# kpreid/all-is-cubes

Measured on AMD Instinct MI355X. Metric: Mrays/s, higher is better.
Workload: dtype f64

## Files before the change

### all_is_cubes_amd/abi.py

```python
from __future__ import annotations

import ctypes as C
import math
from pathlib import Path
from typing import Optional

import numpy as np

_PKG = Path(__file__).resolve().parent
LIB_PATH = _PKG / "libaic_hip.so"

AIC_OK = 0
ERR_NAMES = {1: "AIC_ERR_INVALID", 2: "AIC_ERR_NO_DEVICE", 3: "AIC_ERR_OOM", 4: "AIC_ERR_DEVICE", 5: "AIC_ERR_UNSUPPORTED"}
LAYER_WORLD, LAYER_UI = 0, 1
MAX_IN_FLIGHT = 32
FLAW_UNSUPPORTED, FLAW_NO_BLOOM = 1, 2
FRAME_COUNTERS, FRAME_AUX, FRAME_PIXEL_CENTERS, FRAME_OUT_LINEAR, FRAME_OUT_COLORBUF, FRAME_NO_FEEDBACK = 1, 2, 4, 8, 16, 32
FRAME_BLOOM = 64
RAYS_NO_SKY, RAYS_DEVICE = 128, 256
MAX_RAYS = 2048 * 65535
TUNE_QUEUES_SHIFT, TUNE_SUPER_SHIFT, TUNE_VARIANT_SHIFT = 0, 4, 9
VARIANT_AUTO, VARIANT_PLAIN, VARIANT_EXCHANGING, VARIANT_RECORDING = 0, 1, 2, 3
LIGHT_HOOK_SESSION, LIGHT_HOOK_POOL_SHIFT = 1, 8


def bloom_geometry(width: int, height: int):
    rx, ry = (width + 1) // 2, (height + 1) // 2
    levels = min(6, min(rx, ry).bit_length())
    d = 1 << levels
    return levels, ((rx + d - 1) // d * d, (ry + d - 1) // d * d)


def tuning(queues=None, super_shift=None, variant=None) -> int:
    t = 0
    if queues is not None:
        t |= (int(queues) & 15) << TUNE_QUEUES_SHIFT
    if super_shift is not None:
        t |= ((int(super_shift) + 1) & 31) << TUNE_SUPER_SHIFT
    if variant is not None:
        t |= (int(variant) & 3) << TUNE_VARIANT_SHIFT
    return t

ABI_SYMBOLS = [
    "aic_abi_version", "aic_create", "aic_destroy", "aic_last_error", "aic_device_name", "aic_upload_space",
    "aic_clear_space", "aic_update_cubes", "aic_update_light_volume", "aic_replace_block", "aic_replace_blocks", "aic_compact", "aic_set_options",
    "aic_render", "aic_render_submit", "aic_render_wait", "aic_render_submit_batch", "aic_render_wait_batch", "aic_trace_patches", "aic_trace_rays", "aic_partition_rows", "aic_assemble_strips", "aic_assemble_strips_async", "aic_assemble_strips_on", "aic_read_aux", "aic_synchronize", "aic_stream", "aic_wait_event", "aic_stream_wait_frame",
    "aic_probe_raycast", "aic_probe_light_lut", "aic_probe_powf", "aic_probe_expf", "aic_probe_bloom",
    "aic_ortho_image_size", "aic_render_orthographic",
    "aic_evaluate_light", "aic_evaluate_light_submit", "aic_evaluate_light_wait", "aic_evaluate_light_poll", "aic_light_cubes_changed", "aic_read_light_volume", "aic_read_light_cubes", "aic_light_chart", "aic_probe_derived", "aic_probe_log2f",
    "aic_create_multi", "aic_destroy_multi", "aic_multi_device_count", "aic_multi_context", "aic_multi_last_error", "aic_multi_upload_space",
    "aic_multi_clear_space", "aic_multi_update_cubes", "aic_multi_update_light_volume", "aic_multi_evaluate_light", "aic_multi_light_cubes_changed", "aic_multi_replace_blocks", "aic_multi_set_options",
    "aic_multi_render", "aic_multi_render_submit", "aic_multi_render_wait",
]


class AicError(RuntimeError):

    def __init__(self, code: int, message: str):
        super().__init__(f"{ERR_NAMES.get(code, code)}: {message}")
        self.code = code


class BlockDesc(C.Structure):
    _fields_ = [("resolution", C.c_int32), ("vlo", C.c_int32 * 3), ("vsize", C.c_int32 * 3), ("vox_off", C.c_uint32),
                ("pal_off", C.c_uint32), ("pal_len", C.c_uint32), ("flags", C.c_uint32), ("reserved", C.c_int32)]


class LightParams(C.Structure):
    _fields_ = [("maximum_distance", C.c_int32), ("fast", C.c_int32), ("epsilon", C.c_int32), ("batch", C.c_int32),
                ("queue_order", C.c_int32), ("n_queue", C.c_int32), ("lanes_per_cube", C.c_int32), ("hooks", C.c_int32), ("queue_cubes", C.c_void_p), ("queue_priorities", C.c_void_p),
                ("max_updates", C.c_uint64)]


class LightInfo(C.Structure):
    _fields_ = [("updates", C.c_uint64), ("batches", C.c_uint64), ("cost", C.c_uint64), ("device_ms", C.c_double),
                ("total_ms", C.c_double), ("queue_left", C.c_uint32), ("pad", C.c_uint32), ("bundles_visited", C.c_uint64)]


def light_chart():
    lib = load()
    lib.aic_light_chart.restype = C.c_uint32
    lib.aic_light_chart.argtypes = [C.c_void_p, C.c_void_p, C.POINTER(C.c_uint32)]
    depth = C.c_uint32(0)
    n = lib.aic_light_chart(None, None, C.byref(depth))
    w = np.zeros((n, 6), np.float32)
    ch = np.zeros((n, 6), np.uint32)
    lib.aic_light_chart(w.ctypes.data, ch.ctypes.data, C.byref(depth))
    return w, ch, int(depth.value)


class SpaceDesc(C.Structure):
    _fields_ = [("lo", C.c_int32 * 3), ("size", C.c_int32 * 3), ("block_index", C.c_void_p), ("light", C.c_void_p),
                ("n_blocks", C.c_uint32), ("blocks", C.c_void_p), ("voxels", C.c_void_p), ("n_voxels", C.c_uint64),
                ("palette", C.c_void_p), ("n_palette", C.c_uint64), ("sky_kind", C.c_int32), ("sky", (C.c_float * 3) * 8),
                ("block_sky", (C.c_uint8 * 4) * 7)]


class Options(C.Structure):
    _fields_ = [("fog", C.c_int32), ("transparency", C.c_int32), ("threshold", C.c_float), ("lighting", C.c_int32),
                ("bounce_samples", C.c_int32), ("antialiasing", C.c_int32), ("debug_pixel_cost", C.c_int32),
                ("tone_mapping", C.c_int32), ("maximum_intensity", C.c_float), ("bloom_intensity", C.c_float),
                ("view_distance", C.c_double)]


class Camera(C.Structure):
    _fields_ = [("inverse_projection_view", C.c_double * 16), ("exposure", C.c_float), ("reserved", C.c_int32)]


class Partition(C.Structure):
    _fields_ = [("strip_rows", C.c_uint32), ("n_parts", C.c_uint32), ("part", C.c_uint32), ("reserved", C.c_uint32)]


class FrameDesc(C.Structure):
    _fields_ = [("width", C.c_uint32), ("height", C.c_uint32), ("world", Camera), ("ui", Camera), ("backdrop", C.c_float * 4),
                ("partition", Partition), ("flags", C.c_uint32), ("tuning", C.c_uint32)]


class FrameInfo(C.Structure):
    _fields_ = [("cubes_traced", C.c_uint64), ("n_outer", C.c_uint64), ("n_inner", C.c_uint64), ("n_hits", C.c_uint64),
                ("n_light", C.c_uint64), ("kernel_ms", C.c_float), ("total_ms", C.c_float), ("rows_rendered", C.c_uint32),
                ("flaws", C.c_uint32), ("variant", C.c_uint32), ("tile_queues", C.c_uint32)]


PIXEL_AUX_DTYPE = np.dtype(
    [("hit", "<i4"), ("cube", "<i4", (3,)), ("voxel", "<i4", (3,)), ("resolution", "<i4"), ("face", "<i4"),
     ("block_index", "<i4"), ("cubes_traced", "<u4"), ("layer", "<u4"), ("t_distance", "<f8")],
    align=True,
)
RC_STEP_DTYPE = np.dtype([("cube", "<i4", (3,)), ("face", "<i4"), ("t_distance", "<f8"), ("intersection_point", "<f8", (3,))], align=True)

_lib: Optional[C.CDLL] = None


def load() -> C.CDLL:
    global _lib
    if _lib is None:
        if not LIB_PATH.exists():
            raise ImportError(f"{LIB_PATH} is missing: build it with __graft_entry__.build() (hipcc, gfx950)")
        try:
            import torch
        except ImportError:
            pass
        lib = C.CDLL(str(LIB_PATH))
        lib.aic_create.restype = C.c_void_p
        lib.aic_create.argtypes = [C.c_int, C.POINTER(C.c_int)]
        lib.aic_destroy.argtypes = [C.c_void_p]
        lib.aic_destroy.restype = None
        lib.aic_last_error.restype = C.c_char_p
        lib.aic_last_error.argtypes = [C.c_void_p]
        lib.aic_stream.restype = C.c_void_p
        lib.aic_stream.argtypes = [C.c_void_p]
        lib.aic_partition_rows.restype = C.c_uint32
        lib.aic_partition_rows.argtypes = [C.c_uint32, C.POINTER(Partition)]
        lib.aic_upload_space.argtypes = [C.c_void_p, C.c_int, C.POINTER(SpaceDesc)]
        lib.aic_clear_space.argtypes = [C.c_void_p, C.c_int]
        lib.aic_compact.argtypes = [C.c_void_p, C.c_int]
        lib.aic_update_cubes.argtypes = [C.c_void_p, C.c_int, C.c_uint32, C.c_void_p, C.c_void_p, C.c_void_p]
        lib.aic_update_light_volume.argtypes = [C.c_void_p, C.c_int, C.c_void_p]
        lib.aic_replace_block.argtypes = [C.c_void_p, C.c_int, C.c_uint32, C.POINTER(BlockDesc), C.c_void_p, C.c_void_p]
        lib.aic_replace_blocks.argtypes = [C.c_void_p, C.c_int, C.c_uint32, C.c_void_p, C.c_void_p, C.c_void_p, C.c_void_p]
        lib.aic_set_options.argtypes = [C.c_void_p, C.c_int, C.POINTER(Options)]
        lib.aic_render.argtypes = [C.c_void_p, C.POINTER(FrameDesc), C.c_void_p, C.c_int, C.POINTER(FrameInfo)]
        lib.aic_render_submit.argtypes = [C.c_void_p, C.POINTER(FrameDesc), C.c_void_p, C.c_uint32]
        lib.aic_render_wait.argtypes = [C.c_void_p, C.c_uint32, C.POINTER(FrameInfo)]
        lib.aic_render_submit_batch.argtypes = [C.c_void_p, C.c_uint32, C.POINTER(FrameDesc), C.POINTER(C.c_void_p), C.c_uint32]
        lib.aic_render_wait_batch.argtypes = [C.c_void_p, C.c_uint32, C.c_uint32, C.POINTER(FrameInfo)]
        lib.aic_trace_patches.argtypes = [C.c_void_p, C.POINTER(FrameDesc), C.c_uint32, C.c_void_p, C.c_void_p, C.c_void_p, C.POINTER(FrameInfo)]
        lib.aic_trace_rays.argtypes = [C.c_void_p, C.c_int, C.c_uint32, C.c_void_p, C.c_uint32, C.c_float, C.c_void_p, C.c_void_p, C.POINTER(FrameInfo)]
        lib.aic_assemble_strips.argtypes = [C.c_void_p, C.c_void_p, C.c_void_p, C.c_uint32, C.c_uint32, C.c_uint32, C.c_uint32]
        lib.aic_assemble_strips_async.argtypes = [C.c_void_p, C.c_void_p, C.c_void_p, C.c_uint32, C.c_uint32, C.c_uint32, C.c_uint32]
        lib.aic_read_aux.argtypes = [C.c_void_p, C.c_void_p, C.c_uint64]
        lib.aic_synchronize.argtypes = [C.c_void_p]
        lib.aic_wait_event.argtypes = [C.c_void_p, C.c_void_p]
        lib.aic_stream_wait_frame.argtypes = [C.c_void_p, C.c_uint32, C.c_void_p]
        lib.aic_device_name.argtypes = [C.c_void_p, C.c_char_p, C.c_uint32]
        lib.aic_probe_raycast.argtypes = [C.c_void_p, C.c_void_p, C.c_void_p, C.c_int, C.c_void_p, C.c_void_p, C.c_int,
                                          C.c_uint32, C.c_void_p, C.POINTER(C.c_uint32), C.POINTER(C.c_int)]
        lib.aic_probe_light_lut.argtypes = [C.c_void_p, C.c_void_p]
        lib.aic_probe_powf.argtypes = [C.c_void_p, C.c_void_p, C.c_void_p, C.c_uint32, C.c_void_p]
        lib.aic_probe_expf.argtypes = [C.c_void_p, C.c_void_p, C.c_uint32, C.c_void_p]
        lib.aic_probe_bloom.argtypes = [C.c_void_p, C.c_uint32, C.c_uint32, C.c_void_p, C.c_float, C.POINTER(Options), C.c_void_p, C.c_void_p,
                                        C.POINTER(C.c_uint32 * 2)]
        lib.aic_evaluate_light.argtypes = [C.c_void_p, C.c_int, C.POINTER(LightParams), C.POINTER(LightInfo)]
        lib.aic_evaluate_light_submit.argtypes = [C.c_void_p, C.c_int, C.POINTER(LightParams)]
        lib.aic_evaluate_light_wait.argtypes = [C.c_void_p, C.c_int, C.POINTER(LightInfo)]
        lib.aic_evaluate_light_poll.argtypes = [C.c_void_p, C.c_int, C.POINTER(C.c_int)]
        lib.aic_read_light_volume.argtypes = [C.c_void_p, C.c_int, C.c_void_p]
        lib.aic_read_light_cubes.argtypes = [C.c_void_p, C.c_int, C.c_uint32, C.c_void_p, C.c_void_p]
        lib.aic_light_cubes_changed.argtypes = [C.c_void_p, C.c_int, C.c_uint32, C.c_void_p, C.c_int]
        lib.aic_probe_derived.argtypes = [C.c_void_p, C.c_int, C.c_void_p, C.c_void_p]
        lib.aic_probe_log2f.argtypes = [C.c_void_p, C.c_void_p, C.c_uint32, C.c_void_p]
        assert C.sizeof(BlockDesc) == 48
        _lib = lib
    return _lib


def packed_light_scalar_in(value: float) -> int:
    v = np.float32(value)
    if not v > 0:
        return 0
    x = float(np.float32(np.float32(np.log2(v)) * np.float32(10.0)) + np.float32(144.0))
    x = float(np.float32(x))
    r = math.floor(abs(x) + 0.5) * (1 if x >= 0 else -1)
    return int(min(max(r, 0), 255))


def block_sky_texels(sky_kind: int, sky: np.ndarray) -> np.ndarray:
    sky = np.asarray(sky, np.float32).reshape(8, 3)
    out = np.zeros((7, 4), np.uint8)
    out[:, 3] = 255

    def some(rgb):
        return [packed_light_scalar_in(float(c)) for c in rgb]

    if sky_kind == 0:
        out[:, 0:3] = some(sky[0])
        return out
    bases = {
        0: ((0, 1, 0), (0, 0, 1), (1, 0, 0)),
        1: ((0, 0, 1), (1, 0, 0), (0, 1, 0)),
        2: ((1, 0, 0), (0, 1, 0), (0, 0, 1)),
        3: ((0, -1, 0), (0, 0, 1), (-1, 0, 0)),
        4: ((0, 0, 1), (-1, 0, 0), (0, -1, 0)),
        5: ((1, 0, 0), (0, -1, 0), (0, 0, -1)),
    }
    pts = [(-1, -1, -1), (-1, 1, -1), (1, -1, -1), (1, 1, -1)]
    for f in range(6):
        bx, by, bz = (np.array(v) for v in bases[f])
        acc = np.zeros(3, np.float32)
        for p in pts:
            d = p[0] * bx + p[1] * by + p[2] * bz
            idx = ((1 if d[0] >= 0 else 0) << 2) + ((1 if d[1] >= 0 else 0) << 1) + (1 if d[2] >= 0 else 0)
            acc = (acc + sky[idx]).astype(np.float32)
        out[f, 0:3] = some(acc * np.float32(0.25))
    acc = np.zeros(3, np.float32)
    for k in range(8):
        acc = (acc + sky[k]).astype(np.float32)
    out[6, 0:3] = some(acc * np.float32(1.0 / 8.0))
    return out


def make_options(fog=1, transparency=1, threshold=0.5, lighting=3, bounce_samples=0, antialiasing=0, debug_pixel_cost=False,
                 tone_mapping=0, maximum_intensity=float("inf"), bloom_intensity=0.125, view_distance=200.0) -> Options:
    o = Options()
    o.fog, o.transparency, o.threshold, o.lighting = fog, transparency, threshold, lighting
    o.bounce_samples, o.antialiasing, o.debug_pixel_cost = bounce_samples, antialiasing, int(debug_pixel_cost)
    o.tone_mapping, o.maximum_intensity, o.bloom_intensity = tone_mapping, maximum_intensity, bloom_intensity
    o.view_distance = min(max(view_distance, 1.0), 10000.0)
    return o


def unaltered_colors(**kw) -> Options:
    base = dict(fog=0, lighting=0, transparency=1, bloom_intensity=0.0)
    base.update(kw)
    return make_options(**base)


def _ptr(a: Optional[np.ndarray]):
    return None if a is None or a.size == 0 else a.ctypes.data


# ... 259 lines not shown
            raise ValueError("colorbuf must be [h][w][4]")
        h, w = cb.shape[:2]
        out = np.zeros((h, w, 4), np.uint8)
        size = (C.c_uint32 * 2)()
        t0 = bloom_geometry(w, h)[1]
        mip0 = np.zeros((t0[1], t0[0], 4), np.float16) if want_mip0 else None
        self._check(self._lib.aic_probe_bloom(self._h, w, h, _ptr(cb), float(exposure), C.byref(options), _ptr(out),
                                              _ptr(mip0) if mip0 is not None else None, C.byref(size)))
        assert (size[0], size[1]) == t0, ((size[0], size[1]), t0)
        return (out, mip0) if want_mip0 else out

    def evaluate_light(self, layer: int, maximum_distance: int, fast: bool = True, epsilon: int = 1, batch: int = 32,
                       queue_order: int = 16, queue=None, max_updates: int = 0, lanes_per_cube: int = 0, session: bool = False,
                       dep_pool_chunks: int = 0) -> LightInfo:
        hooks = (LIGHT_HOOK_SESSION if session else 0) | ((int(dep_pool_chunks) & 0xffff) << LIGHT_HOOK_POOL_SHIFT)
        p = LightParams(maximum_distance, int(fast), epsilon, batch, queue_order, -1, lanes_per_cube, hooks, None, None, max_updates)
        keep = []
        if queue is not None:
            qc = np.ascontiguousarray([q[0] for q in queue], np.int32).reshape(-1, 3)
            qp = np.ascontiguousarray([q[1] for q in queue], np.int32)
            keep = [qc, qp]
            p.n_queue = len(qp)
            p.queue_cubes = qc.ctypes.data
            p.queue_priorities = qp.ctypes.data
        info = LightInfo()
        self._check(self._lib.aic_evaluate_light(self._h, layer, C.byref(p), C.byref(info)))
        del keep
        return info

    def evaluate_light_submit(self, layer: int, maximum_distance: int, fast: bool = True, epsilon: int = 1, batch: int = 32, queue_order: int = 16,
                              queue=None, max_updates: int = 0, lanes_per_cube: int = 0) -> None:
        p = LightParams(maximum_distance, int(fast), epsilon, batch, queue_order, -1, lanes_per_cube, 0, None, None, max_updates)
        keep = []
        if queue is not None:
            qc = np.ascontiguousarray([q[0] for q in queue], np.int32).reshape(-1, 3)
            qp = np.ascontiguousarray([q[1] for q in queue], np.int32)
            keep = [qc, qp]
            p.n_queue = len(qp)
            p.queue_cubes = qc.ctypes.data
            p.queue_priorities = qp.ctypes.data
        self._check(self._lib.aic_evaluate_light_submit(self._h, layer, C.byref(p)))
        del keep

    def evaluate_light_done(self, layer: int) -> bool:
        d = C.c_int(1)
        self._check(self._lib.aic_evaluate_light_poll(self._h, layer, C.byref(d)))
        return bool(d.value)

    def evaluate_light_wait(self, layer: int) -> LightInfo:
        info = LightInfo()
        self._check(self._lib.aic_evaluate_light_wait(self._h, layer, C.byref(info)))
        return info

    def light_cubes_changed(self, layer: int, xyz, queue_order: int = 16) -> None:
        xyz = np.ascontiguousarray(xyz, np.int32).reshape(-1, 3)
        self._check(self._lib.aic_light_cubes_changed(self._h, layer, len(xyz), _ptr(xyz), queue_order))

    def read_light_volume(self, layer: int, shape) -> np.ndarray:
        out = np.zeros(tuple(shape) + (4,), np.uint8)
        self._check(self._lib.aic_read_light_volume(self._h, layer, out.ctypes.data))
        return out

    def read_light_cubes(self, layer: int, xyz) -> np.ndarray:
        xyz = np.ascontiguousarray(xyz, np.int32).reshape(-1, 3)
        out = np.zeros((len(xyz), 4), np.uint8)
        self._check(self._lib.aic_read_light_cubes(self._h, layer, len(xyz), _ptr(xyz), out.ctypes.data))
        return out

    def probe_derived(self, layer: int, n_blocks: int):
        out = np.zeros((n_blocks, 32), np.float32)
        opq = np.zeros((n_blocks, 6), np.uint8)
        self._check(self._lib.aic_probe_derived(self._h, layer, out.ctypes.data, opq.ctypes.data))
        return out, opq

    def probe_log2f(self, x) -> np.ndarray:
        x = np.ascontiguousarray(x, np.float32)
        out = np.zeros(x.shape, np.float32)
        self._check(self._lib.aic_probe_log2f(self._h, _ptr(x), x.size, _ptr(out)))
        return out

    def probe_light_lut(self) -> np.ndarray:
        out = np.zeros(256, np.float32)
        self._check(self._lib.aic_probe_light_lut(self._h, out.ctypes.data))
        return out


class MultiContext:

    def __init__(self, device_ids):
        self._lib = load()
        lib = self._lib
        lib.aic_create_multi.restype = C.c_void_p
        lib.aic_create_multi.argtypes = [C.c_int, C.c_void_p, C.POINTER(C.c_int)]
        lib.aic_destroy_multi.argtypes = [C.c_void_p]
        lib.aic_multi_last_error.restype = C.c_char_p
        lib.aic_multi_last_error.argtypes = [C.c_void_p]
        lib.aic_multi_device_count.argtypes = [C.c_void_p]
        lib.aic_multi_upload_space.argtypes = [C.c_void_p, C.c_int, C.c_void_p]
        lib.aic_multi_clear_space.argtypes = [C.c_void_p, C.c_int]
        lib.aic_multi_set_options.argtypes = [C.c_void_p, C.c_int, C.c_void_p]
        lib.aic_multi_update_light_volume.argtypes = [C.c_void_p, C.c_int, C.c_void_p]
        lib.aic_multi_evaluate_light.argtypes = [C.c_void_p, C.c_int, C.POINTER(LightParams), C.POINTER(LightInfo)]
        lib.aic_multi_light_cubes_changed.argtypes = [C.c_void_p, C.c_int, C.c_uint32, C.c_void_p, C.c_int]
        lib.aic_multi_update_cubes.argtypes = [C.c_void_p, C.c_int, C.c_uint32, C.c_void_p, C.c_void_p, C.c_void_p]
        lib.aic_multi_render.argtypes = [C.c_void_p, C.c_void_p, C.c_void_p, C.c_int, C.c_void_p]
        lib.aic_multi_render_submit.argtypes = [C.c_void_p, C.c_void_p, C.c_void_p, C.c_int, C.c_uint32]
        lib.aic_multi_render_wait.argtypes = [C.c_void_p, C.c_uint32, C.c_void_p]
        ids = np.ascontiguousarray(device_ids, np.int32)
        st = C.c_int(0)
        self._h = lib.aic_create_multi(len(ids), _ptr(ids), C.byref(st))
        if not self._h:
            raise AicError(st.value, "aic_create_multi failed (no usable MI355X?)")

    def close(self) -> None:
        if self._h:
            self._lib.aic_destroy_multi(self._h)
            self._h = None

    def __enter__(self):
        return self

    def __exit__(self, *exc):
        self.close()

    def _check(self, rc: int) -> None:
        if rc != AIC_OK:
            raise AicError(rc, self._lib.aic_multi_last_error(self._h).decode())

    @property
    def device_count(self) -> int:
        return int(self._lib.aic_multi_device_count(self._h))

    def upload_space(self, layer: int, flat_space) -> None:
        d, _keep = Context._space_desc(flat_space)
        self._check(self._lib.aic_multi_upload_space(self._h, layer, C.byref(d)))

    def clear_space(self, layer: int) -> None:
        self._check(self._lib.aic_multi_clear_space(self._h, layer))

    def set_options(self, layer: int, options: Options) -> None:
        self._check(self._lib.aic_multi_set_options(self._h, layer, C.byref(options)))

    def update_light_volume(self, layer: int, light) -> None:
        lt = np.ascontiguousarray(light, np.uint8)
        self._check(self._lib.aic_multi_update_light_volume(self._h, layer, _ptr(lt)))

    def evaluate_light(self, layer: int, maximum_distance: int, fast: bool = True, epsilon: int = 1, batch: int = 32, queue_order: int = 16) -> LightInfo:
        p = LightParams(maximum_distance, int(fast), epsilon, batch, queue_order, -1, 0, 0, None, None, 0)
        info = LightInfo()
        self._check(self._lib.aic_multi_evaluate_light(self._h, layer, C.byref(p), C.byref(info)))
        return info

    def light_cubes_changed(self, layer: int, xyz, queue_order: int = 16) -> None:
        xyz = np.ascontiguousarray(xyz, np.int32).reshape(-1, 3)
        self._check(self._lib.aic_multi_light_cubes_changed(self._h, layer, len(xyz), _ptr(xyz), queue_order))

    def update_cubes(self, layer: int, xyz, block_index=None, light=None) -> None:
        xyz = np.ascontiguousarray(xyz, np.int32).reshape(-1, 3)
        bi = None if block_index is None else np.ascontiguousarray(block_index, np.uint16)
        lt = None if light is None else np.ascontiguousarray(light, np.uint8).reshape(-1, 4)
        self._check(self._lib.aic_multi_update_cubes(self._h, layer, len(xyz), _ptr(xyz), _ptr(bi), _ptr(lt)))

    def render(self, frame: FrameDesc):
        out = np.zeros((frame.height, frame.width, 4), np.uint8)
        info = FrameInfo()
        self._check(self._lib.aic_multi_render(self._h, C.byref(frame), _ptr(out), 0, C.byref(info)))
# ... 12 lines not shown
```

### all_is_cubes_amd/csrc/aic_abi.cpp

```cpp

#include <hip/hip_runtime.h>

#include <chrono>
#include <cmath>
#include <condition_variable>
#include <mutex>
#include <thread>
#include <cstdio>
#include <cstdlib>
#include <cstring>
#include <initializer_list>
#include <string>
#include <utility>
#include <vector>

#include "../../include/aic_hip.h"
#include "aic_bloom.h"
#include "aic_ctx.h"
#include "aic_device.h"

namespace aic {
void launch_trace_image(const DevFrame &F, bool diag, hipStream_t stream);
size_t trace_ray_cold_bytes(uint32_t n_cus, uint32_t *groups);
void launch_scatter_cubes(uint16_t *grid, uint32_t *light, const int32_t *xyz, const uint16_t *bi, const uint32_t *lt,
                          uint32_t n, const int lo[3], const int size[3], const uint32_t *cls, hipStream_t stream);
void launch_probe_powf(const float *x, const float *y, float *out, uint32_t n, hipStream_t stream);
void launch_probe_expf(const float *x, float *out, uint32_t n, hipStream_t stream);
void launch_order_tiles(const uint32_t *cost, uint32_t *order, uint32_t n_tiles, uint32_t macros_x, uint32_t sb_shift, uint32_t n_queues, uint32_t *queue_start,
                        hipStream_t stream, bool clear_cost = false, uint32_t *clear_words = nullptr, uint32_t n_clear_words = 0);
void launch_order_tiles_jobs(const OrderJobs &jobs, uint32_t n_jobs, uint32_t n_tiles, uint32_t macros_x, uint32_t sb_shift, uint32_t n_queues, hipStream_t stream,
                             bool clear_cost, uint32_t n_clear_words);
void launch_tag_cubes(uint16_t *grid, size_t n, const uint32_t *cls, int from_tagged, int to_tagged, hipStream_t stream);
void launch_assemble_strips(const uint32_t *gathered, uint32_t *out, uint32_t w, uint32_t h, uint32_t strip_rows,
                            uint32_t n_parts, uint32_t max_rows, hipStream_t stream);
void launch_probe_raycast(const double *od, int use_bounds, const int *lohi, int include_exit, uint32_t max_steps,
                          double *out_rec, uint32_t *n_out, int *ended, hipStream_t stream);
}

using namespace aic;

static_assert(sizeof(aic_pixel_aux) == sizeof(DevAux), "aux record layout");

static_assert(sizeof(aic_block_desc) == 48, "aic_block_desc is 48 bytes");

namespace {

constexpr uint64_t kMaxPoolElems = 0x7ffffff0ull;
constexpr uint64_t kMaxLightTexels = 0x3ffffff0ull;

aic_options default_options() {
    aic_options o;
    std::memset(&o, 0, sizeof(o));
    o.fog = 1;
    o.transparency = 1;
    o.threshold = 0.5f;
    o.lighting = 3;
    o.maximum_intensity = INFINITY;
    o.bloom_intensity = 0.125f;
    o.view_distance = 200.0;
    return o;
}

enum DumpTag : uint32_t { DUMP_UPLOAD = 1, DUMP_CLEAR = 2, DUMP_CUBES = 3, DUMP_LIGHT = 4, DUMP_BLOCK = 5, DUMP_OPTIONS = 6, DUMP_FRAME = 7 };
struct DumpPart { const void *p; size_t n; };
void dump_record(aic_ctx *c, uint32_t tag, uint32_t layer, std::initializer_list<DumpPart> parts) {
    if (!c || !c->dump) return;
    uint64_t total = 0;
    for (const DumpPart &d : parts) total += d.p ? d.n : 0;
    std::fwrite(&tag, 4, 1, c->dump);
    std::fwrite(&layer, 4, 1, c->dump);
    std::fwrite(&total, 8, 1, c->dump);
    for (const DumpPart &d : parts)
        if (d.p && d.n) std::fwrite(d.p, 1, d.n, c->dump);
    std::fflush(c->dump);
}

}

namespace aic {

thread_local std::string *tl_err_sink = nullptr;
int fail(aic_ctx *c, int code, const char *what, hipError_t e) {
    if (c) {
        std::string &dst = tl_err_sink ? *tl_err_sink : c->err;
        dst = what;
        if (e != hipSuccess) {
            dst += ": ";
            dst += hipGetErrorString(e);
        }
    }
    return code;
}

int hip_fail(aic_ctx *c, const char *what, hipError_t e) {
    return fail(c, e == hipErrorOutOfMemory ? AIC_ERR_OOM : AIC_ERR_DEVICE, what, e);
}

int take_light_spare(aic_ctx *c, Layer &l, int layer, size_t n, int *index) {
    auto in_use = [&](const DevBuf<uint32_t> &b) {
        for (uint32_t i = 0; i < AIC_MAX_IN_FLIGHT; i++)
            if (c->slots[i].busy && b.p && c->slots[i].light_used[layer] == (const void *)b.p) return true;
        return false;
    };
    int pick = -1;
    for (int k = 0; k < Layer::kLightSpares && pick < 0; k++)
        if (l.light_spare[k].p && l.light_spare[k].cap >= n && !in_use(l.light_spare[k])) pick = k;
    for (int k = 0; k < Layer::kLightSpares && pick < 0; k++)
        if (!l.light_spare[k].p || (l.light_spare[k].cap < n && !in_use(l.light_spare[k]))) pick = k;
    if (pick < 0) {
        pick = 0;
        for (uint32_t i = 0; i < AIC_MAX_IN_FLIGHT; i++)
            if (c->slots[i].busy && c->slots[i].light_used[layer] == (const void *)l.light_spare[0].p) {
                const hipError_t e = hipStreamSynchronize(c->slots[i].stream);
                if (e != hipSuccess) return fail(c, AIC_ERR_DEVICE, "waiting for a frame that reads a spare light volume", e);
            }
    }
    const hipError_t e = l.light_spare[pick].ensure(n);
    if (e != hipSuccess) return fail(c, e == hipErrorOutOfMemory ? AIC_ERR_OOM : AIC_ERR_DEVICE, "alloc light (spare volume)", e);
    *index = pick;
    return AIC_OK;
}

int quiesce(aic_ctx *c) {
    { const int rc = light_job_finish(c); if (rc != AIC_OK) return rc; }
    for (uint32_t i = 0; i < AIC_MAX_IN_FLIGHT; i++)
        if (c->slots[i].busy) HIP_TRY(c, hipStreamSynchronize(c->slots[i].stream));
// ... 73 lines not shown
    for (size_t i = 0; i < nvox; i++) {
        uint16_t idx = voxels[i];
        if (idx >= d.pal_len) return fail(c, AIC_ERR_INVALID, "voxel index exceeds palette");
        (*vox_out)[vox_base + i] = (uint16_t)remap[idx];
    }
    out->kind = (uint32_t)d.resolution;
    out->vlo_packed = (uint32_t)d.vlo[0] | ((uint32_t)d.vlo[1] << 8) | ((uint32_t)d.vlo[2] << 16);
    out->vsize_packed = (uint32_t)d.vsize[0] | ((uint32_t)d.vsize[1] << 8) | ((uint32_t)d.vsize[2] << 16);
    out->vox_off = vox_off;
    out->pal_off = pal_off;
    out->n_invisible = n_inv;
    return AIC_OK;
}

void fill_dev_layer(const aic_ctx *c, const Layer &l, const aic_camera &cam, DevLayer *d, uint32_t *flaws) {
    std::memset(d, 0, sizeof(*d));
    d->present = l.present ? 1 : 0;
    d->pool = l.pool.p;
    d->cls = l.cls.p;
    d->n_blocks = (uint32_t)l.host_blocks.size();
    d->light = l.light.p;
    d->blocks = l.blocks.p;
    d->palette = l.palette.p;
    for (int a = 0; a < 3; a++) { d->lo[a] = l.lo[a]; d->size[a] = l.size[a]; }
    d->air_index = l.air_index;
    d->sky_kind = l.sky_kind;
    std::memcpy(d->sky, l.sky, sizeof(d->sky));
    std::memcpy(d->block_sky, l.block_sky, sizeof(d->block_sky));
    const aic_options o = l.opt_set ? l.opt : default_options();
    d->opt.fog = o.fog;
    d->opt.transparency = o.transparency;
    d->opt.threshold = o.threshold;
    d->opt.lighting = o.lighting;
    d->opt.bounce_samples = o.bounce_samples;
    d->opt.antialiasing = o.antialiasing;
    d->opt.debug_pixel_cost = o.debug_pixel_cost;
    d->opt.tone_mapping = o.tone_mapping;
    d->opt.maximum_intensity = o.maximum_intensity;
    d->opt.view_distance = o.view_distance;
    std::memcpy(d->inv, cam.inverse_projection_view, sizeof(d->inv));
    d->exposure = cam.exposure + 0.0f;
    d->cls_in_code = l.cls_in_code ? 1u : 0u;
    (void)c;
}

}

extern "C" {

int aic_abi_version(void) { return AIC_ABI_VERSION; }

aic_ctx *aic_create(int device_id, int *status) {
    int st_dummy;
    if (!status) status = &st_dummy;
    int n = 0;
    hipError_t e = hipGetDeviceCount(&n);
    if (e != hipSuccess || n <= 0) {
        *status = AIC_ERR_NO_DEVICE;
        return nullptr;
    }
    if (device_id < 0) {
        if (hipGetDevice(&device_id) != hipSuccess) device_id = 0;
    }
    if (device_id >= n) {
        *status = AIC_ERR_INVALID;
        return nullptr;
    }
    if (hipSetDevice(device_id) != hipSuccess) {
        *status = AIC_ERR_DEVICE;
        return nullptr;
    }
    aic_ctx *c = new aic_ctx();
    c->device = device_id;
    hipDeviceProp_t prop;
    if (hipGetDeviceProperties(&prop, device_id) == hipSuccess) c->n_cus = prop.multiProcessorCount > 0 ? (uint32_t)prop.multiProcessorCount : 256u;
    if (hipGetDeviceProperties(&prop, device_id) == hipSuccess) std::snprintf(c->devname, sizeof(c->devname), "%s (%s)", prop.name, prop.gcnArchName);
    {
        auto env_int = [](const char *name, int dflt) { const char *e = std::getenv(name); return e ? std::atoi(e) : dflt; };
        c->sw.tile = env_int("AIC_TILE", 0);
        c->sw.macro = env_int("AIC_MACRO", 0);
        c->sw.feedback = env_int("AIC_TILE_FEEDBACK", 1) != 0;
        c->sw.wait_whole_stream = env_int("AIC_WAIT_WHOLE_STREAM", 0) != 0;
        c->sw.tiles_per_wave = (uint32_t)std::max(0, env_int("AIC_TILES_PER_WAVE", 0));
        if (const char *p = std::getenv("AIC_WAVE_PROF")) c->sw.wave_prof = p;
    }
    if (const char *path = std::getenv("AIC_DUMP")) {
        static int n_dumps = 0;
        std::string pth = path;
        if (n_dumps > 0) pth += "." + std::to_string(n_dumps);
        n_dumps++;
        c->dump = std::fopen(pth.c_str(), "wb");
        if (c->dump) std::fwrite("AICDUMP1", 1, 8, c->dump);
    }
    bool ok = hipStreamCreateWithFlags(&c->stream, hipStreamNonBlocking) == hipSuccess;
    for (uint32_t i = 0; ok && i < 8u && i < AIC_MAX_IN_FLIGHT; i++) {
        aic_ctx::FrameSlot &fs = c->slots[i];
        if (i == 0) fs.stream = c->stream;
        else ok = hipStreamCreateWithFlags(&fs.stream, hipStreamNonBlocking) == hipSuccess;
        ok = ok && hipEventCreate(&fs.ev0) == hipSuccess && hipEventCreate(&fs.ev1) == hipSuccess && hipEventCreate(&fs.ev2) == hipSuccess && fs.sub[0].counters.ensure(1) == hipSuccess;
    }
    ok = ok && hipStreamCreateWithFlags(&c->upload_stream, hipStreamNonBlocking) == hipSuccess;
    float lut[256];
    lut[0] = 0.f;
    for (int v = 1; v < 256; v++) {
        float arg = ((float)v - 144.0f) / 10.0f;
        lut[v] = (float)std::exp2((double)arg);
    }
    ok = ok && c->lut.ensure(256) == hipSuccess && hipMemcpy(c->lut.p, lut, sizeof(lut), hipMemcpyHostToDevice) == hipSuccess;
    {
        auto enc = [](float cc) -> int {
            float v = cc <= 0.0031308f ? cc * (323.f / 25.f) : (211.f * std::pow(cc, 5.f / 12.f) - 11.f) / 200.f;
            float r = std::round(v * 255.f);
            if (!(r > 0.f)) return 0;
            return r >= 255.f ? 255 : (int)r;
        };
        float thr[256];
        thr[0] = 0.f;
        for (int k = 1; k < 256; k++) {
            uint32_t lo_b = 0u, hi_b = 0x40000000u;
            while (hi_b - lo_b > 1u) {
                const uint32_t mid = lo_b + (hi_b - lo_b) / 2u;
                float f;
                std::memcpy(&f, &mid, 4);
                if (enc(f) >= k) hi_b = mid; else lo_b = mid;
            }
            for (int back = 0; back < 8 && hi_b > 1u; back++) {
                uint32_t probe = hi_b - 1u;
                float f;
                std::memcpy(&f, &probe, 4);
                bool lower_found = false;
                for (uint32_t d = 0; d < 8u && probe > d; d++) {
                    const uint32_t q = probe - d;
                    std::memcpy(&f, &q, 4);
                    if (enc(f) >= k) { hi_b = q; lower_found = true; }
                }
                if (!lower_found) break;
            }
            std::memcpy(&thr[k], &hi_b, 4);
        }
        ok = ok && c->srgb_thr.ensure(256) == hipSuccess && hipMemcpy(c->srgb_thr.p, thr, sizeof(thr), hipMemcpyHostToDevice) == hipSuccess;
    }
    if (!ok) {
        *status = AIC_ERR_DEVICE;
        aic_destroy(c);
        return nullptr;
    }
    for (auto &l : c->layers) l.opt = default_options();
    *status = AIC_OK;
    return c;
}

void aic_destroy(aic_ctx *c) {
    if (!c) return;
    (void)hipSetDevice(c->device);
    (void)light_job_finish(c);
    if (c->ljob.worker.joinable()) {
        { std::lock_guard<std::mutex> lk(c->ljob.mu); c->ljob.quit = true; }
        c->ljob.cv.notify_all();
        c->ljob.worker.join();
    }
    if (c->stream) (void)hipStreamSynchronize(c->stream);
    for (uint32_t i = 0; i < AIC_MAX_IN_FLIGHT; i++) {
        aic_ctx::FrameSlot &fs = c->slots[i];
        if (fs.stream) (void)hipStreamSynchronize(fs.stream);
        for (auto &sb : fs.sub) sb.release();
        fs.ray_cold.release(); fs.edges.release();
        if (fs.ev0) (void)hipEventDestroy(fs.ev0);
        if (fs.ev1) (void)hipEventDestroy(fs.ev1);
        if (fs.ev2) (void)hipEventDestroy(fs.ev2);
        fs.tile_static.release(); fs.queue_static.release();
        if (i > 0 && fs.stream) (void)hipStreamDestroy(fs.stream);
    }
    for (auto &l : c->layers) l.release();
    c->lut.release(); c->srgb_thr.release(); c->out.release(); c->aux.release(); c->staging.release(); c->ortho_views.release();
    if (c->dump) std::fclose(c->dump);
    if (c->upload_stream) (void)hipStreamDestroy(c->upload_stream);
    if (c->stream) (void)hipStreamDestroy(c->stream);
    delete c;
}

const char *aic_last_error(const aic_ctx *c) { return c ? c->err.c_str() : "no context"; }

int aic_device_name(const aic_ctx *c, char *buf, uint32_t buf_len) {
    if (!c || !buf || !buf_len) return AIC_ERR_INVALID;
    std::snprintf(buf, buf_len, "%s", c->devname);
    return AIC_OK;
}

int aic_upload_space(aic_ctx *c, int layer, const aic_space_desc *s) {
    if (!c || !s || !valid_layer(layer)) return fail(c, AIC_ERR_INVALID, "aic_upload_space: bad argument");
    HIP_TRY(c, hipSetDevice(c->device));
    { int qrc = quiesce(c); if (qrc != AIC_OK) return qrc; }
    for (int a = 0; a < 3; a++)
        if (s->size[a] < 0 || (int64_t)s->lo[a] + s->size[a] > 2147483647LL) return fail(c, AIC_ERR_INVALID, "space bounds out of range");
    Layer &l = c->layers[layer];
    const size_t n = (size_t)s->size[0] * (size_t)s->size[1] * (size_t)s->size[2];
    if (n && (!s->block_index || !s->light)) return fail(c, AIC_ERR_INVALID, "space has cubes but no block_index/light");
    if (s->n_blocks > 65536) return fail(c, AIC_ERR_INVALID, "more than 65536 blocks");
    if (n + s->n_voxels > kMaxPoolElems) return fail(c, AIC_ERR_INVALID, "space too large (cube grid + voxel pool must stay within 4 GiB)");
    if (n > kMaxLightTexels) return fail(c, AIC_ERR_INVALID, "space too large (the light volume, 4 bytes per cube, must stay within 4 GiB)");
    if (s->n_blocks && !s->blocks) return fail(c, AIC_ERR_INVALID, "blocks is null");
    for (int o = 0; o < 8; o++)
        for (int k = 0; k < 3; k++)
            if (!(s->sky[o][k] >= 0.f)) return fail(c, AIC_ERR_INVALID, "sky colour has a negative or NaN component");

    std::vector<DevBlock> blocks(s->n_blocks);
    std::vector<uint32_t> vox_cap(s->n_blocks, 0u), pal_cap(s->n_blocks, 0u), vox_base(s->n_blocks, 0u), pal_base(s->n_blocks, 0u);
    std::vector<uint16_t> vox;
    std::vector<DevPaletteEntry> pal;
    vox.reserve((size_t)s->n_voxels);
    pal.reserve((size_t)s->n_palette);
    int32_t air_index = -1;
    for (uint32_t i = 0; i < s->n_blocks; i++) {
        const aic_block_desc &d = s->blocks[i];
        const bool one = (d.flags & AIC_BLOCK_ONE) != 0;
        size_t nvox = one ? 1 : (size_t)(d.vsize[0] > 0 ? d.vsize[0] : 0) * (size_t)(d.vsize[1] > 0 ? d.vsize[1] : 0) * (size_t)(d.vsize[2] > 0 ? d.vsize[2] : 0);
        if ((uint64_t)d.vox_off + nvox > s->n_voxels || (uint64_t)d.pal_off + d.pal_len > s->n_palette)
            return fail(c, AIC_ERR_INVALID, "block voxel/palette range exceeds the pools");
        if (n + vox.size() + nvox > kMaxPoolElems || pal.size() + d.pal_len > 0xfffffff0ull) return fail(c, AIC_ERR_INVALID, "pool too large");
        const size_t vb = vox.size(), pb = pal.size();
        int rc = convert_block(c, d, s->voxels ? s->voxels + d.vox_off : nullptr, s->palette ? s->palette + 8 * (size_t)d.pal_off : nullptr,
                               (uint32_t)(n + vox.size()), (uint32_t)pal.size(), &blocks[i], &vox, &pal);
        if (rc != AIC_OK) return rc;
        vox_cap[i] = (uint32_t)(vox.size() - vb);
        pal_cap[i] = (uint32_t)(pal.size() - pb);
        vox_base[i] = (uint32_t)(n + vb);
        pal_base[i] = (uint32_t)pb;
        if ((d.flags & AIC_BLOCK_AIR) && air_index < 0) air_index = (int32_t)i;
    }
    for (size_t i = 0; i < n; i++)
        if (s->block_index[i] >= s->n_blocks) return fail(c, AIC_ERR_INVALID, "cube block index out of range");

    hipError_t e;
    std::vector<uint32_t> cls;
    for (uint32_t i = 0; i < s->n_blocks; i++) set_class(cls, i, block_class(blocks[i]));
    if (cls.empty()) cls.push_back(0u);
    if ((e = l.pool.ensure(n + vox.size())) != hipSuccess) return hip_fail(c, "alloc pool", e);
    if ((e = l.cls.ensure(cls.size())) != hipSuccess) return hip_fail(c, "alloc classes", e);
    if ((e = l.light.ensure(n)) != hipSuccess) return hip_fail(c, "alloc light", e);
    if ((e = l.blocks.ensure(blocks.size())) != hipSuccess) return hip_fail(c, "alloc blocks", e);
    if ((e = l.palette.ensure(pal.size())) != hipSuccess) return hip_fail(c, "alloc palette", e);
    if (n) {
        HIP_TRY(c, hipMemcpyAsync(l.pool.p, s->block_index, n * sizeof(uint16_t), hipMemcpyHostToDevice, c->stream));
        HIP_TRY(c, hipMemcpyAsync(l.light.p, s->light, n * 4, hipMemcpyHostToDevice, c->stream));
    }
    if (!blocks.empty()) HIP_TRY(c, hipMemcpyAsync(l.blocks.p, blocks.data(), blocks.size() * sizeof(DevBlock), hipMemcpyHostToDevice, c->stream));
    if (!vox.empty()) HIP_TRY(c, hipMemcpyAsync(l.pool.p + n, vox.data(), vox.size() * sizeof(uint16_t), hipMemcpyHostToDevice, c->stream));
    HIP_TRY(c, hipMemcpyAsync(l.cls.p, cls.data(), cls.size() * sizeof(uint32_t), hipMemcpyHostToDevice, c->stream));
    const bool cls_in_code = s->n_blocks <= kCubeIndexMask + 1u;
    if (cls_in_code) launch_tag_cubes(l.pool.p, n, l.cls.p, 0, 1, c->stream);
    if (!pal.empty()) HIP_TRY(c, hipMemcpyAsync(l.palette.p, pal.data(), pal.size() * sizeof(DevPaletteEntry), hipMemcpyHostToDevice, c->stream));
    HIP_TRY(c, hipStreamSynchronize(c->stream));

    for (int a = 0; a < 3; a++) { l.lo[a] = s->lo[a]; l.size[a] = s->size[a]; }
// ... 303 lines not shown
    const double *rays;
    uint32_t n;
    bool no_sky;
    uint32_t layer;
    DevAux *aux_target;
};
int submit_frames(aic_ctx *c, uint32_t k, const aic_frame_desc *frames, uint32_t *const *out_devices, uint32_t slot, bool allow_aux, const double *patches = nullptr,
                  uint32_t n_patches = 0, const DevOrthoView *ortho = nullptr, int32_t ortho_n = 0, const RayBatch *rb = nullptr) {
    if (rb) n_patches = rb->n;
    aic_ctx::FrameSlot &fs = c->slots[slot];
    const aic_frame_desc *f = &frames[0];
    fs.t_begin = std::chrono::steady_clock::now();
    fs.n_sub = k;
    aic_partition part = f->partition;
    if (part.n_parts <= 1 || part.strip_rows == 0) {
        part.n_parts = 1;
        part.part = 0;
        part.strip_rows = f->height ? f->height : 1;
    }
    if (part.part >= part.n_parts) return fail(c, AIC_ERR_INVALID, "aic_render: partition.part >= n_parts");
    if (f->flags & AIC_FRAME_BLOOM) {
        if (f->flags & (AIC_FRAME_OUT_LINEAR | AIC_FRAME_OUT_COLORBUF)) return fail(c, AIC_ERR_INVALID, "aic_render: AIC_FRAME_BLOOM is for RGBA8 output only");
        if (part.n_parts > 1u) return fail(c, AIC_ERR_UNSUPPORTED, "aic_render: AIC_FRAME_BLOOM needs the whole frame (partition.n_parts = 1)");
        if (patches || ortho_n || rb) return fail(c, AIC_ERR_UNSUPPORTED, "AIC_FRAME_BLOOM: not for patches, rays or orthographic views");
    }
    const uint32_t local_rows = aic_partition_rows(f->height, &part);
    const size_t npix = (size_t)f->width * local_rows;
    for (uint32_t j = 0; j < k; j++)
        if (npix && !out_devices[j]) return fail(c, AIC_ERR_INVALID, "aic_render: output buffer is null");
    if (!patches && !rb)
        for (uint32_t j = 0; j < k; j++) dump_record(c, DUMP_FRAME, slot, {{&frames[j], sizeof(frames[j])}});
    if (f->width > 65535u || local_rows > 65535u) return fail(c, AIC_ERR_INVALID, "aic_render: frame dimensions above 65535 are not supported");
    for (uint32_t j = 0; j < k; j++)
        if (!(frames[j].world.exposure >= 0.f) || !(frames[j].ui.exposure >= 0.f)) return fail(c, AIC_ERR_INVALID, "aic_render: exposure is negative or NaN");

    uint32_t flaws = 0;
    DevFrame F;
    std::memset(&F, 0, sizeof(F));
    DevLayer hl[2];
    fill_dev_layer(c, c->layers[AIC_LAYER_WORLD], f->world, &hl[0], &flaws);
    fill_dev_layer(c, c->layers[AIC_LAYER_UI], f->ui, &hl[1], &flaws);
    const aic_options &bloom_opt = c->layers[AIC_LAYER_WORLD].opt;
    const bool bloom = (f->flags & AIC_FRAME_BLOOM) && bloom_opt.bloom_intensity > 0.0f;
    if (bloom_opt.bloom_intensity != 0.0f && !bloom) flaws |= AIC_FLAW_NO_BLOOM;
    F.width = f->width;
    F.height = f->height;
    F.n_sub = k;
    F.pixel_centers = (f->flags & AIC_FRAME_PIXEL_CENTERS) && !patches ? 1 : 0;
    F.out_mode = (f->flags & AIC_FRAME_OUT_LINEAR) ? 1 : ((f->flags & AIC_FRAME_OUT_COLORBUF) || bloom ? 2 : 0);
    F.patches = patches;
    F.n_patches = n_patches;
    F.ortho = ortho;
    F.ortho_n = ortho_n;
    F.rays = rb ? rb->rays : nullptr;
    F.bare_trace = (ortho_n || rb) ? 1 : 0;
    if (rb) hl[1].present = 0;
    if (ortho_n) {
        hl[1].present = 0;
        DevOptions &o = hl[0].opt;
        o.fog = 0; o.transparency = 1; o.lighting = 0; o.antialiasing = 0; o.debug_pixel_cost = 0; o.tone_mapping = 0;
        o.maximum_intensity = INFINITY; o.view_distance = 200.0;
        hl[0].exposure = 1.0f;
        flaws = 0;
    }
    F.antialias = (hl[0].opt.antialiasing == 2 && !F.pixel_centers && !rb) ? 1 : 0;
    F.maximum_intensity = hl[0].opt.maximum_intensity;
    F.tone_mapping = hl[0].opt.tone_mapping;
    F.strip_rows = part.strip_rows;
    F.n_parts = part.n_parts;
    F.part = part.part;
    F.local_rows = local_rows;
    {
        const int forced = c->sw.tile;
        F.tile = (forced == 8 || forced == 16) ? (uint32_t)forced : 8u;
        F.tiles_x = (f->width + F.tile - 1) / F.tile;
        F.tiles_y = (local_rows + F.tile - 1) / F.tile;
        const int macro_env = c->sw.macro;
        F.macro = (macro_env == 1 || macro_env == 2 || macro_env == 4 || macro_env == 8 || macro_env == 16) ? (uint32_t)macro_env : 2u;
        F.macros_x = (F.tiles_x + F.macro - 1) / F.macro;
        F.macros_y = (F.tiles_y + F.macro - 1) / F.macro;
    }
    F.light_lut = c->lut.p;
    F.n_cus = c->n_cus;
    F.tiles_per_wave = c->sw.tiles_per_wave ? c->sw.tiles_per_wave : (c->streaming_submit ? 4u : 1u);
    if (!c->sw.tiles_per_wave && c->streaming_submit && k == 1u) {
        uint32_t busy_others = 0;
        for (uint32_t i = 0; i < AIC_MAX_IN_FLIGHT; i++) busy_others += (i != slot && c->slots[i].busy) ? 1u : 0u;
        const uint32_t resident_waves = (uint32_t)c->n_cus * 16u;
        const uint32_t tpw_full = (F.tiles_x * F.tiles_y + resident_waves - 1u) / resident_waves;
        if (tpw_full >= 4u && busy_others > 0u) {
            const uint32_t t = tpw_full * (busy_others < 4u ? busy_others : 4u);
            F.tiles_per_wave = t < 32u ? t : (tpw_full > 32u ? tpw_full : 32u);
        }
    }
    F.srgb_thr = c->srgb_thr.p;

    const bool want_aux = allow_aux && (f->flags & AIC_FRAME_AUX) != 0;
    const bool diag = want_aux || (f->flags & AIC_FRAME_COUNTERS) != 0;
    fs.diag = diag;
    fs.flaws = flaws;
    fs.light_used[0] = hl[0].light;
    fs.light_used[1] = hl[1].light;
    fs.local_rows = local_rows;
    fs.npix = npix;
    fs.variant = fs.tile_queues = 0;
    if (allow_aux) c->aux_records = 0;
    if (!npix) return AIC_OK;
    hipError_t e;
    if (want_aux) {
        if (rb && rb->aux_target) {
            F.aux = rb->aux_target;
        } else {
            if ((e = c->aux.ensure(npix)) != hipSuccess) return hip_fail(c, "alloc aux", e);
            F.aux = c->aux.p;
        }
    }
    const bool ui = hl[1].present != 0;
    const uint32_t n_tiles = F.macros_x * F.macros_y;
    const int queues_env = (int)((f->tuning >> AIC_TUNE_QUEUES_SHIFT) & 15u);
    const int super_env = (int)((f->tuning >> AIC_TUNE_SUPER_SHIFT) & 31u) - 1;
    uint32_t n_queues = queues_env > 0 ? (uint32_t)queues_env : (uint32_t)c->n_cus / 32u;
    if (n_queues > kMaxTileQueues) n_queues = kMaxTileQueues;
    if (n_queues < 2u || patches || rb || ortho_n || !n_tiles) n_queues = 0u;
    const uint32_t macro_log2 = F.macro >= 16 ? 4u : (F.macro >= 8 ? 3u : (F.macro >= 4 ? 2u : (F.macro >= 2 ? 1u : 0u)));
    const uint32_t tile_log2 = F.tile >= 16 ? 4u : 3u;
    uint32_t sb_px_log2 = 0;
    while ((2u << sb_px_log2) <= std::max(1u, local_rows / 8u)) sb_px_log2++;
    const uint32_t sb_shift = super_env >= 0 ? (uint32_t)std::min(super_env, 12) : (sb_px_log2 > macro_log2 + tile_log2 ? sb_px_log2 - macro_log2 - tile_log2 : 0u);
    const bool use_feedback = c->sw.feedback && n_tiles && !patches && !rb && !ortho_n && !(f->flags & AIC_FRAME_NO_FEEDBACK);
    const uint32_t sig[4] = {f->width, local_rows, (part.n_parts << 16) | part.part, (part.strip_rows << 8) | (F.macro << 4) | (F.tile >> 3)};
    uint32_t order_key[6] = {sig[0], sig[1], sig[2], sig[3], n_queues, sb_shift};
    const bool ordered = use_feedback || n_queues;
    F.n_queues = ordered ? n_queues : 0u;
    if (ordered && n_queues) {
        bool any_static = false;
        for (uint32_t j = 0; j < k; j++) {
            aic_ctx::SubSlot &sb = fs.sub[j];
            const bool same = use_feedback && sb.record_ready && std::memcmp(order_key, sb.order_key, sizeof(order_key)) == 0 && sb.tile_order.n >= n_tiles &&
                              cameras_close(frames[j].world.inverse_projection_view, sb.cost_cam);
            any_static = any_static || !same;
        }
        if (any_static && (!fs.static_ready || std::memcmp(order_key, fs.static_key, sizeof(order_key)) != 0 || fs.tile_static.n < n_tiles)) {
            fs.static_ready = false;
            if ((e = fs.tile_static.ensure(n_tiles)) != hipSuccess || (e = fs.queue_static.ensure(kMaxTileQueues + 1)) != hipSuccess) return hip_fail(c, "alloc tile queues", e);
            launch_order_tiles(nullptr, fs.tile_static.p, n_tiles, F.macros_x, sb_shift, n_queues, fs.queue_static.p, fs.stream);
            HIP_TRY(c, hipGetLastError());
            std::memcpy(fs.static_key, order_key, sizeof(order_key));
            fs.static_ready = true;
        }
    }
    for (uint32_t j = 0; j < k; j++) {
        aic_ctx::SubSlot &sb = fs.sub[j];
        DevSub &S = F.sub[j];
        std::memcpy(S.backdrop, frames[j].backdrop, sizeof(S.backdrop));
        S.has_backdrop = !(frames[j].backdrop[0] == 0.f && frames[j].backdrop[1] == 0.f && frames[j].backdrop[2] == 0.f && frames[j].backdrop[3] == 0.f);
        S.exposure = ortho_n ? 1.0f : frames[j].world.exposure + 0.0f;
        S.out = out_devices[j];
        if (bloom) {
            if ((e = sb.bloom_cb.ensure(npix)) != hipSuccess || (e = sb.bloom_mips.ensure(bloom_geometry(f->width, f->height).texels)) != hipSuccess)
                return hip_fail(c, "alloc bloom scratch", e);
            S.out = reinterpret_cast<uint32_t *>(sb.bloom_cb.p);
        }
        if ((e = sb.counters.ensure(1)) != hipSuccess) return hip_fail(c, "alloc frame counters", e);
        S.counters = sb.counters.p;
        if (!sb.host_counters) {
            HIP_TRY(c, hipHostMalloc((void **)&sb.host_counters, sizeof(DevCounters), hipHostMallocDefault));
            std::memset(sb.host_counters, 0, sizeof(DevCounters));
        }
        if (!sb.counters_clean) HIP_TRY(c, hipMemsetAsync(sb.counters.p, 0, sizeof(DevCounters), fs.stream));
        sb.counters_clean = false;
        if (ordered) {
            bool same = use_feedback && sb.record_ready && std::memcmp(order_key, sb.order_key, sizeof(order_key)) == 0 && sb.tile_order.n >= n_tiles;
            if (same) {
                same = cameras_close(frames[j].world.inverse_projection_view, sb.cost_cam);
// ... 8 lines not shown
            if (use_feedback) {
                const uint32_t *const before = sb.tile_cost.p;
                if ((e = sb.tile_cost.ensure(n_tiles)) != hipSuccess) return hip_fail(c, "alloc tile feedback", e);
                if (sb.tile_cost.p != before) sb.cost_clean_n = 0;
                if (sb.cost_clean_n < n_tiles) HIP_TRY(c, hipMemsetAsync(sb.tile_cost.p, 0, (size_t)n_tiles * sizeof(uint32_t), fs.stream));
                sb.cost_clean_n = 0;
                S.tile_cost = sb.tile_cost.p;
                std::memcpy(sb.cost_sig, sig, sizeof(sig));
            }
        }
        if (ui) {
            const size_t samples = F.antialias ? 4 : 1;
            if ((e = sb.acc.ensure(samples * npix)) != hipSuccess) return hip_fail(c, "alloc accumulators", e);
            S.acc_buf = sb.acc.p;
        }
    }
    if (!patches && !rb && !ortho_n) {
        if (fs.edges_w != f->width || fs.edges_h != f->height || !fs.edges.p) {
            std::vector<double> host((size_t)f->width + 1 + (size_t)f->height + 1);
            for (uint32_t x = 0; x <= f->width; x++) host[x] = ((double)x) / (double)f->width * 2.0 - 1.0;
            for (uint32_t y = 0; y <= f->height; y++) host[(size_t)f->width + 1 + y] = -(((double)y) / (double)f->height * 2.0 - 1.0);
            fs.edges_w = fs.edges_h = 0;
            if ((e = fs.edges.ensure(host.size())) != hipSuccess) return hip_fail(c, "alloc pixel edges", e);
            HIP_TRY(c, hipMemcpyAsync(fs.edges.p, host.data(), host.size() * sizeof(double), hipMemcpyHostToDevice, fs.stream));
            HIP_TRY(c, hipStreamSynchronize(fs.stream));
            fs.edges_w = f->width; fs.edges_h = f->height;
        }
        F.edge_x = fs.edges.p;
        F.edge_y = fs.edges.p + (size_t)f->width + 1;
    }
    if (!diag) {
        uint32_t groups = 0;
        const size_t bytes = trace_ray_cold_bytes(c->n_cus, &groups);
        if (bytes) {
            const uint32_t asked = (f->tuning >> AIC_TUNE_VARIANT_SHIFT) & 3u;
            const double resident_waves = (double)c->n_cus * 16.0 / (double)k;
            const double need = c->streaming_submit ? 1.9 : 5.0;
            F.exchange = asked == AIC_VARIANT_EXCHANGING ? 1u : (asked == AIC_VARIANT_PLAIN ? 0u : (((double)F.tiles_x * (double)F.tiles_y >= need * resident_waves) ? 1u : 0u));
            if (F.exchange && F.antialias) {
                if ((e = fs.ray_cold.ensure(bytes / sizeof(uint4))) != hipSuccess) return hip_fail(c, "alloc ray state", e);
                F.ray_cold = fs.ray_cold.p;
                F.ray_cold_groups = groups;
            }
        }
    }
    HIP_TRY(c, hipEventRecord(fs.ev0, fs.stream));
    if (ui) {
        F.pass = 1;
        F.hit_layer = 1u;
        F.use_init = 0;
        F.layer = hl[1];
        F.layer_transparency = hl[1].opt.transparency;
        F.layer_lighting = hl[1].opt.lighting;
        DevSub keep[kMaxSub];
        std::memcpy(keep, F.sub, sizeof(keep));
        const uint32_t queues_keep = F.n_queues;
        for (uint32_t j = 0; j < k; j++) {
            std::memcpy(F.sub[j].inv, frames[j].ui.inverse_projection_view, sizeof(F.sub[j].inv));
            F.sub[j].tile_order = nullptr;
            F.sub[j].tile_cost = nullptr;
            F.sub[j].queue_start = nullptr;
            F.sub[j].host_counters = nullptr;
        }
        F.n_queues = 0u;
        launch_trace_image(F, diag, fs.stream);
        std::memcpy(F.sub, keep, sizeof(keep));
        F.n_queues = queues_keep;
        for (uint32_t j = 0; j < k; j++) HIP_TRY(c, hipMemsetAsync(&fs.sub[j].counters.p->tile_next, 0, sizeof(uint32_t), fs.stream));
        F.use_init = 1;
    }
    F.pass = (rb && rb->no_sky) ? 2 : 0;
    F.hit_layer = rb ? rb->layer : 0u;
    for (uint32_t j = 0; j < k; j++) {
        std::memcpy(F.sub[j].inv, ortho_n ? hl[0].inv : frames[j].world.inverse_projection_view, sizeof(F.sub[j].inv));
#ifndef AIC_PROFILE
        F.sub[j].host_counters = reinterpret_cast<unsigned long long *>(fs.sub[j].host_counters);
#endif
    }
    F.layer = hl[0];
    F.layer_transparency = hl[0].opt.transparency;
    F.layer_lighting = hl[0].opt.lighting;
    fs.variant = diag ? AIC_VARIANT_RECORDING : ((F.exchange && hl[0].opt.lighting != 5 && (F.ray_cold || !F.antialias)) ? AIC_VARIANT_EXCHANGING : AIC_VARIANT_PLAIN);
    fs.tile_queues = F.n_queues;
    launch_trace_image(F, diag, fs.stream);
    HIP_TRY(c, hipGetLastError());
    if (bloom) {
        const BloomGeom geom = bloom_geometry(f->width, f->height);
        for (uint32_t j = 0; j < k; j++) {
            BloomParams bp;
            bp.colorbuf = fs.sub[j].bloom_cb.p;
            bp.mips = fs.sub[j].bloom_mips.p;
            bp.out = out_devices[j];
            bp.exposure = F.sub[j].exposure;
            bp.intensity = bloom_opt.bloom_intensity;
            bp.tone_mapping = F.tone_mapping;
            bp.maximum_intensity = F.maximum_intensity;
            bp.srgb_thr = c->srgb_thr.p;
            launch_bloom(geom, bp, fs.stream);
        }
        HIP_TRY(c, hipGetLastError());
    }
    HIP_TRY(c, hipEventRecord(fs.ev1, fs.stream));
#ifdef AIC_PROFILE
    for (uint32_t j = 0; j < k; j++) HIP_TRY(c, hipMemcpyAsync(fs.sub[j].host_counters, fs.sub[j].counters.p, sizeof(DevCounters), hipMemcpyDeviceToHost, fs.stream));
#endif
    HIP_TRY(c, hipEventRecord(fs.ev2, fs.stream));
    fs.busy = true;
    bool cleared = false;
    if (use_feedback && n_tiles) {
        OrderJobs jobs;
        std::memset(&jobs, 0, sizeof(jobs));
        bool ok = true;
        for (uint32_t j = 0; j < k; j++) {
            aic_ctx::SubSlot &sb = fs.sub[j];
            sb.record_ready = false;
            sb.cost_clean_n = 0;
            ok = ok && sb.tile_order.ensure(n_tiles) == hipSuccess && sb.queue_start.ensure(kMaxTileQueues + 1) == hipSuccess;
            jobs.cost[j] = sb.tile_cost.p; jobs.order[j] = sb.tile_order.p; jobs.queue_start[j] = sb.queue_start.p;
            jobs.clear_words[j] = reinterpret_cast<uint32_t *>(sb.counters.p);
        }
        if (ok) {
            launch_order_tiles_jobs(jobs, k, n_tiles, F.macros_x, sb_shift, n_queues ? n_queues : 1u, fs.stream, true, (uint32_t)(sizeof(DevCounters) / 4));
            if (hipGetLastError() == hipSuccess) {
                cleared = true;
                for (uint32_t j = 0; j < k; j++) {
                    aic_ctx::SubSlot &sb = fs.sub[j];
                    sb.cost_clean_n = n_tiles;
                    std::memcpy(sb.order_key, order_key, sizeof(order_key));
                    std::memcpy(sb.cost_cam, frames[j].world.inverse_projection_view, sizeof(sb.cost_cam));
                    sb.record_ready = true;
                }
            }
        }
    }
    if (!cleared) {
        cleared = true;
        for (uint32_t j = 0; j < k; j++) cleared = (hipMemsetAsync(fs.sub[j].counters.p, 0, sizeof(DevCounters), fs.stream) == hipSuccess) && cleared;
    }
    for (uint32_t j = 0; j < k; j++) fs.sub[j].counters_clean = cleared;
    if (want_aux && !(rb && rb->aux_target)) c->aux_records = npix;
    return AIC_OK;
}
int submit_frame(aic_ctx *c, const aic_frame_desc *f, uint32_t *out_device, uint32_t slot, bool allow_aux, const double *patches = nullptr,
                 uint32_t n_patches = 0, const DevOrthoView *ortho = nullptr, int32_t ortho_n = 0) {
    uint32_t *const outs[1] = {out_device};
    return submit_frames(c, 1, f, outs, slot, allow_aux, patches, n_patches, ortho, ortho_n);
}

int wait_frame(aic_ctx *c, uint32_t slot, aic_frame_info *info, bool whole_stream = false, aic_frame_info *infos = nullptr, uint32_t n_infos = 0) {
    aic_ctx::FrameSlot &fs = c->slots[slot];
    if (info) std::memset(info, 0, sizeof(*info));
    for (uint32_t j = 0; infos && j < n_infos; j++) std::memset(&infos[j], 0, sizeof(infos[j]));
    float kernel_ms = 0.f;
    const uint32_t k = fs.n_sub ? fs.n_sub : 1u;
    if (fs.busy) {
        fs.busy = false;
        if (whole_stream || c->sw.wait_whole_stream) HIP_TRY(c, hipStreamSynchronize(fs.stream));
        else HIP_TRY(c, hipEventSynchronize(fs.ev2));
        HIP_TRY(c, hipEventElapsedTime(&kernel_ms, fs.ev0, fs.ev1));
        for (uint32_t j = 0; j < k; j++) {
            DevCounters hc;
            std::memcpy(&hc, fs.sub[j].host_counters, sizeof(hc));
            if (hc.bailed) return fail(c, AIC_ERR_DEVICE, "trace kernel: a wave gave up waiting for rays in transit between waves; the frame has unwritten pixels");
            if (info) {
                info->cubes_traced += hc.cubes_traced;
                info->n_outer += hc.n_outer;
                info->n_inner += hc.n_inner;
                info->n_hits += hc.n_hits;
                info->n_light += hc.n_light;
            }
            if (infos && j < n_infos) {
                infos[j].cubes_traced = hc.cubes_traced; infos[j].n_outer = hc.n_outer; infos[j].n_inner = hc.n_inner;
                infos[j].n_hits = hc.n_hits; infos[j].n_light = hc.n_light;
            }
#ifdef AIC_PROFILE
            { static const char *names[40] = {"max_lifetime","max_until_dry","cyc_until_dry","cyc_lifetime","shade_ph","shade_ln","enter_ph","enter_ln","ray_ph","ray_ln","step_iters","step_lanes","cyc_step","cyc_shade_rest","cyc_enter","cyc_newray","cyc_finish","cyc_refill","cyc_shade_light","cyc_sched","fast_iters","fast_lanes","trips","trip_lanes","pass_hl_lanes","pass_fast_eligible","leave_blocks","leave_lanes","apply_blocks","apply_lanes","pass_needed_lanes","xchg_rounds","xchg_lanes","cyc_xchg","xchg_picked","xchg_parked","idle_spins","xchg_claims_lost","xchg_empty","-"};
              if (!fs.diag) for (int i = 0; i < 39; i++) std::fprintf(stderr, "PROF %s %llu\n", names[i], hc.prof[i]);
              if (const char *path = (fs.diag || c->sw.wave_prof.empty()) ? nullptr : c->sw.wave_prof.c_str()) {
                  if (FILE *fp = std::fopen(path, "w")) {
                      for (int w = 0; w < 2048; w++) std::fprintf(fp, "%u %u %u %u\n", hc.wave_prof[w][0], hc.wave_prof[w][1], hc.wave_prof[w][2], hc.wave_prof[w][3]);
                      std::fclose(fp);
                  }
              } }
#endif
        }
    }
    const float total_ms = std::chrono::duration<float, std::milli>(std::chrono::steady_clock::now() - fs.t_begin).count();
    auto fill = [&](aic_frame_info *o) {
        o->kernel_ms = kernel_ms;
        o->rows_rendered = fs.local_rows;
        o->flaws = fs.flaws;
        o->variant = fs.npix ? fs.variant : 0u;
        o->tile_queues = fs.npix ? fs.tile_queues : 0u;
        o->total_ms = total_ms;
    };
    if (info) fill(info);
    for (uint32_t j = 0; infos && j < n_infos && j < k; j++) fill(&infos[j]);
    return AIC_OK;
}

}

int aic_render(aic_ctx *c, const aic_frame_desc *f, void *out_rgba8, int out_is_device, aic_frame_info *info) {
    if (!c || !f) return fail(c, AIC_ERR_INVALID, "aic_render: bad argument");
    if (info) std::memset(info, 0, sizeof(*info));
    HIP_TRY(c, hipSetDevice(c->device));
    if (c->slots[0].busy) return fail(c, AIC_ERR_INVALID, "aic_render: a submitted frame still occupies slot 0 (aic_render_wait it first)");
    uint32_t *target = (uint32_t *)out_rgba8;
    const size_t px_words = (f->flags & (AIC_FRAME_OUT_LINEAR | AIC_FRAME_OUT_COLORBUF)) ? 4 : 1;
    if (!out_is_device && out_rgba8) {
        aic_partition part = f->partition;
        if (part.n_parts <= 1 || part.strip_rows == 0) { part.n_parts = 1; part.part = 0; part.strip_rows = f->height ? f->height : 1; }
        const size_t npix = (size_t)f->width * (part.part < part.n_parts ? aic_partition_rows(f->height, &part) : 0);
        hipError_t e;
        if (npix && (e = c->out.ensure(npix * px_words)) != hipSuccess) return hip_fail(c, "alloc output", e);
        target = c->out.p;
    }
    int rc = submit_frame(c, f, target, 0, true);
    if (rc != AIC_OK) return rc;
    if (!out_is_device && c->slots[0].npix)
        HIP_TRY(c, hipMemcpyAsync(out_rgba8, c->out.p, c->slots[0].npix * px_words * 4, hipMemcpyDeviceToHost, c->slots[0].stream));
    return wait_frame(c, 0, info, !out_is_device);
}

namespace {

struct Mat4h { double m[16]; };
Mat4h mat_identity() { Mat4h t{}; t.m[0] = t.m[5] = t.m[10] = t.m[15] = 1.0; return t; }
Mat4h mat_then(const Mat4h &a, const Mat4h &b) {
    Mat4h o{};
    for (int r = 0; r < 4; r++)
        for (int cc = 0; cc < 4; cc++)
            o.m[r * 4 + cc] = a.m[r * 4 + 0] * b.m[0 * 4 + cc] + a.m[r * 4 + 1] * b.m[1 * 4 + cc] + a.m[r * 4 + 2] * b.m[2 * 4 + cc] + a.m[r * 4 + 3] * b.m[3 * 4 + cc];
    return o;
}
void ortho_view(int resolution, const int32_t lo[3], const int32_t size[3], int viewed_face , DevOrthoView *out) {
    const int axis = (viewed_face - 1) % 3;
    const int32_t ub[3] = {lo[0] + size[0], lo[1] + size[1], lo[2] + size[2]};
    out->w = (uint32_t)(axis == 0 ? size[2] : size[0]) * (uint32_t)resolution;
    out->h = (uint32_t)(axis == 1 ? size[2] : size[1]) * (uint32_t)resolution;
    double ot[3];
    int bx[3], by[3], bz[3];
    auto set = [](int v[3], int x, int y, int z) { v[0] = x; v[1] = y; v[2] = z; };
    switch (viewed_face) {
        case 1: ot[0] = lo[0]; ot[1] = ub[1]; ot[2] = lo[2]; set(bx, 0, 0, 1); set(by, 0, 1, 0); set(bz, -1, 0, 0); break;
// ... 93 lines not shown
                      aic_frame_info *info) {
    if (!c || !f || (n && (!rects || !out_rgba8))) return fail(c, AIC_ERR_INVALID, "aic_trace_patches: bad argument");
    if (info) std::memset(info, 0, sizeof(*info));
    if (!n) return AIC_OK;
    HIP_TRY(c, hipSetDevice(c->device));
    if (c->slots[0].busy) return fail(c, AIC_ERR_INVALID, "aic_trace_patches: a submitted frame still occupies slot 0 (aic_render_wait it first)");
    if (f->flags & AIC_FRAME_BLOOM) return fail(c, AIC_ERR_UNSUPPORTED, "aic_trace_patches: AIC_FRAME_BLOOM needs a whole frame");
    aic_frame_desc g = *f;
    g.width = n < 2048u ? n : 2048u;
    g.height = (n + g.width - 1u) / g.width;
    if (g.height > 65535u) return fail(c, AIC_ERR_INVALID, "aic_trace_patches: more than 2048 x 65535 rectangles in one call");
    g.partition = aic_partition{0, 1, 0, 0};
    g.flags = (f->flags & (AIC_FRAME_COUNTERS | AIC_FRAME_OUT_LINEAR | AIC_FRAME_OUT_COLORBUF)) | (aux ? AIC_FRAME_AUX : 0u);
    const size_t npix = (size_t)g.width * g.height;
    hipError_t e;
    const size_t px_words = (f->flags & (AIC_FRAME_OUT_LINEAR | AIC_FRAME_OUT_COLORBUF)) ? 4 : 1;
    if ((e = c->out.ensure(npix * px_words)) != hipSuccess) return hip_fail(c, "alloc output", e);
    if ((e = c->staging.ensure((size_t)n * 32)) != hipSuccess) return hip_fail(c, "alloc staging", e);
    HIP_TRY(c, hipMemcpyAsync(c->staging.p, rects, (size_t)n * 32, hipMemcpyHostToDevice, c->slots[0].stream));
    int rc = submit_frame(c, &g, c->out.p, 0, true, (const double *)c->staging.p, n);
    if (rc != AIC_OK) return rc;
    HIP_TRY(c, hipMemcpyAsync(out_rgba8, c->out.p, (size_t)n * px_words * 4, hipMemcpyDeviceToHost, c->slots[0].stream));
    rc = wait_frame(c, 0, info, true);
    if (rc != AIC_OK) return rc;
    if (aux) {
        HIP_TRY(c, hipMemcpy(aux, c->aux.p, (size_t)n * sizeof(aic_pixel_aux), hipMemcpyDeviceToHost));
    }
    if (info) info->rows_rendered = n;
    return AIC_OK;
}

int aic_trace_rays(aic_ctx *c, int layer, uint32_t n, const double *rays, uint32_t flags, float exposure, void *out, aic_pixel_aux *aux,
                   aic_frame_info *info) {
    if (!c || !valid_layer(layer) || (n && (!rays || !out))) return fail(c, AIC_ERR_INVALID, "aic_trace_rays: bad argument");
    if (info) std::memset(info, 0, sizeof(*info));
    if (flags & AIC_FRAME_BLOOM) return fail(c, AIC_ERR_UNSUPPORTED, "aic_trace_rays: AIC_FRAME_BLOOM needs a whole frame");
    if ((flags & AIC_FRAME_OUT_LINEAR) && (flags & AIC_FRAME_OUT_COLORBUF)) return fail(c, AIC_ERR_INVALID, "aic_trace_rays: AIC_FRAME_OUT_LINEAR and AIC_FRAME_OUT_COLORBUF exclude each other");
    if (!(exposure >= 0.f)) return fail(c, AIC_ERR_INVALID, "aic_trace_rays: exposure is negative or NaN");
    if (!n) return AIC_OK;
    HIP_TRY(c, hipSetDevice(c->device));
    if (c->slots[0].busy) return fail(c, AIC_ERR_INVALID, "aic_trace_rays: a submitted frame still occupies slot 0 (aic_render_wait it first)");
    if (!c->layers[layer].present) return fail(c, AIC_ERR_INVALID, "aic_trace_rays: no space uploaded for this layer");
    const bool on_device = (flags & AIC_RAYS_DEVICE) != 0;
    const size_t px_words = (flags & (AIC_FRAME_OUT_LINEAR | AIC_FRAME_OUT_COLORBUF)) ? 4 : 1;
    if (on_device && (((uintptr_t)rays & 15u) || ((uintptr_t)out & (px_words * 4u - 1u)) || ((uintptr_t)aux & 7u)))
        return fail(c, AIC_ERR_INVALID, "aic_trace_rays: AIC_RAYS_DEVICE wants rays at a 16-byte boundary, out and aux at their element's");
    aic_frame_desc g;
    std::memset(&g, 0, sizeof(g));
    g.width = n < 2048u ? n : 2048u;
    g.height = (n + g.width - 1u) / g.width;
    if (g.height > 65535u) return fail(c, AIC_ERR_INVALID, "aic_trace_rays: more than 2048 x 65535 rays in one call");
    g.partition = aic_partition{0, 1, 0, 0};
    g.flags = (flags & (AIC_FRAME_COUNTERS | AIC_FRAME_OUT_LINEAR | AIC_FRAME_OUT_COLORBUF)) | (aux ? AIC_FRAME_AUX : 0u);
    g.tuning = flags & (3u << AIC_TUNE_VARIANT_SHIFT);
    g.world.exposure = exposure;
    g.ui.exposure = 1.0f;
    hipError_t e;
    RayBatch rb{rays, n, (flags & AIC_RAYS_NO_SKY) != 0, (uint32_t)layer, on_device ? reinterpret_cast<DevAux *>(aux) : nullptr};
    uint32_t *target = (uint32_t *)out;
    hipStream_t stream = c->slots[0].stream;
    if (!on_device) {
        if ((e = c->out.ensure((size_t)n * px_words)) != hipSuccess) return hip_fail(c, "alloc output", e);
        if ((e = c->staging.ensure((size_t)n * 48)) != hipSuccess) return hip_fail(c, "alloc staging", e);
        HIP_TRY(c, hipMemcpyAsync(c->staging.p, rays, (size_t)n * 48, hipMemcpyHostToDevice, stream));
        rb.rays = (const double *)c->staging.p;
        target = c->out.p;
    }
    const bool swap_layers = layer != AIC_LAYER_WORLD;
    if (swap_layers) std::swap(c->layers[AIC_LAYER_WORLD], c->layers[layer]);
    int rc = submit_frames(c, 1, &g, &target, 0, true, nullptr, 0, nullptr, 0, &rb);
    if (swap_layers) std::swap(c->layers[AIC_LAYER_WORLD], c->layers[layer]);
    if (rc != AIC_OK) return rc;
    if (!on_device) HIP_TRY(c, hipMemcpyAsync(out, c->out.p, (size_t)n * px_words * 4, hipMemcpyDeviceToHost, stream));
    rc = wait_frame(c, 0, info, !on_device);
    if (rc != AIC_OK) return rc;
    if (aux && !on_device) HIP_TRY(c, hipMemcpy(aux, c->aux.p, (size_t)n * sizeof(aic_pixel_aux), hipMemcpyDeviceToHost));
    if (info) info->rows_rendered = n;
    return AIC_OK;
}

static int ensure_slot(aic_ctx *c, uint32_t slot) {
    aic_ctx::FrameSlot &fs = c->slots[slot];
    if (fs.stream && fs.ev0 && fs.ev1 && fs.ev2 && fs.sub[0].counters.p) return AIC_OK;
    if (!fs.stream) {
        HIP_TRY(c, hipStreamCreateWithFlags(&fs.stream, hipStreamNonBlocking));
        hipEvent_t ev = nullptr;
        HIP_TRY(c, hipEventCreateWithFlags(&ev, hipEventDisableTiming));
        hipError_t e1 = hipEventRecord(ev, c->stream);
        if (e1 == hipSuccess) e1 = hipStreamWaitEvent(fs.stream, ev, 0);
        (void)hipEventDestroy(ev);
        if (e1 != hipSuccess) return hip_fail(c, "order a new slot's stream behind the context's waits", e1);
    }
    if (!fs.ev0) HIP_TRY(c, hipEventCreate(&fs.ev0));
    if (!fs.ev1) HIP_TRY(c, hipEventCreate(&fs.ev1));
    if (!fs.ev2) HIP_TRY(c, hipEventCreate(&fs.ev2));
    hipError_t e = fs.sub[0].counters.ensure(1);
    if (e != hipSuccess) return hip_fail(c, "alloc frame counters", e);
    return AIC_OK;
}

int aic_render_submit(aic_ctx *c, const aic_frame_desc *f, void *out_device, uint32_t slot) {
    if (!c || !f || slot >= AIC_MAX_IN_FLIGHT) return fail(c, AIC_ERR_INVALID, "aic_render_submit: bad argument");
    HIP_TRY(c, hipSetDevice(c->device));
    if (c->slots[slot].busy) return fail(c, AIC_ERR_INVALID, "aic_render_submit: slot busy (aic_render_wait it first)");
    { const int rs = ensure_slot(c, slot); if (rs != AIC_OK) return rs; }
    c->streaming_submit = true;
    const int rc = submit_frame(c, f, (uint32_t *)out_device, slot, false);
    c->streaming_submit = false;
    return rc;
}

int aic_render_submit_batch(aic_ctx *c, uint32_t n_frames, const aic_frame_desc *frames, void *const *out_devices, uint32_t slot) {
    if (!c || !frames || !out_devices || slot >= AIC_MAX_IN_FLIGHT) return fail(c, AIC_ERR_INVALID, "aic_render_submit_batch: bad argument");
    if (n_frames != 1u && n_frames != 2u && n_frames != 4u && n_frames != 8u) return fail(c, AIC_ERR_INVALID, "aic_render_submit_batch: 1, 2, 4 or 8 frames per launch");
    for (uint32_t j = 1; j < n_frames; j++) {
        const aic_frame_desc &a = frames[0], &b = frames[j];
        if (a.width != b.width || a.height != b.height || a.flags != b.flags || a.tuning != b.tuning || std::memcmp(&a.partition, &b.partition, sizeof(a.partition)) != 0)
            return fail(c, AIC_ERR_INVALID, "aic_render_submit_batch: the frames of a batch share size, partition, flags and tuning");
    }
    HIP_TRY(c, hipSetDevice(c->device));
    if (c->slots[slot].busy) return fail(c, AIC_ERR_INVALID, "aic_render_submit_batch: slot busy (aic_render_wait it first)");
    { const int rs = ensure_slot(c, slot); if (rs != AIC_OK) return rs; }
    uint32_t *outs[kMaxSub];
    for (uint32_t j = 0; j < n_frames; j++) outs[j] = (uint32_t *)out_devices[j];
    c->streaming_submit = true;
    const int rc = submit_frames(c, n_frames, frames, outs, slot, false);
    c->streaming_submit = false;
    return rc;
}

int aic_render_wait(aic_ctx *c, uint32_t slot, aic_frame_info *info) {
    if (!c || slot >= AIC_MAX_IN_FLIGHT) return fail(c, AIC_ERR_INVALID, "aic_render_wait: bad argument");
    HIP_TRY(c, hipSetDevice(c->device));
    return wait_frame(c, slot, info);
}

int aic_render_wait_batch(aic_ctx *c, uint32_t slot, uint32_t n_frames, aic_frame_info *infos) {
    if (!c || slot >= AIC_MAX_IN_FLIGHT || (n_frames && !infos)) return fail(c, AIC_ERR_INVALID, "aic_render_wait_batch: bad argument");
    HIP_TRY(c, hipSetDevice(c->device));
    return wait_frame(c, slot, nullptr, false, infos, n_frames);
}

int aic_assemble_strips_on(aic_ctx *c, const void *gathered_device, void *out_device, uint32_t width, uint32_t height,
                           uint32_t strip_rows, uint32_t n_parts, void *hip_stream) {
    if (!c || !gathered_device || !out_device || !strip_rows || !n_parts) return fail(c, AIC_ERR_INVALID, "aic_assemble_strips: bad argument");
    HIP_TRY(c, hipSetDevice(c->device));
    uint32_t max_rows = 0;
    for (uint32_t p = 0; p < n_parts; p++) {
        aic_partition pp = {strip_rows, n_parts, p, 0};
        uint32_t r = aic_partition_rows(height, &pp);
        if (r > max_rows) max_rows = r;
    }
    launch_assemble_strips((const uint32_t *)gathered_device, (uint32_t *)out_device, width, height, strip_rows, n_parts, max_rows, hip_stream ? (hipStream_t)hip_stream : c->stream);
    HIP_TRY(c, hipGetLastError());
    return AIC_OK;
}

int aic_assemble_strips_async(aic_ctx *c, const void *gathered_device, void *out_device, uint32_t width, uint32_t height,
                              uint32_t strip_rows, uint32_t n_parts) {
    return aic_assemble_strips_on(c, gathered_device, out_device, width, height, strip_rows, n_parts, nullptr);
}

int aic_assemble_strips(aic_ctx *c, const void *gathered_device, void *out_device, uint32_t width, uint32_t height,
                        uint32_t strip_rows, uint32_t n_parts) {
    const int rc = aic_assemble_strips_async(c, gathered_device, out_device, width, height, strip_rows, n_parts);
    if (rc != AIC_OK) return rc;
    HIP_TRY(c, hipStreamSynchronize(c->stream));
    return AIC_OK;
// ... 62 lines not shown
    uint32_t n = 0;
    int en = 0;
    HIP_TRY(c, hipMemcpyAsync(&n, d_n, 4, hipMemcpyDeviceToHost, c->stream));
    HIP_TRY(c, hipMemcpyAsync(&en, d_end, 4, hipMemcpyDeviceToHost, c->stream));
    if (max_steps) HIP_TRY(c, hipMemcpyAsync(rec.data(), d_rec, rec.size() * sizeof(double), hipMemcpyDeviceToHost, c->stream));
    HIP_TRY(c, hipStreamSynchronize(c->stream));
    for (uint32_t i = 0; i < n && i < max_steps; i++) {
        const double *r = rec.data() + 8 * (size_t)i;
        out[i].cube[0] = (int32_t)r[0]; out[i].cube[1] = (int32_t)r[1]; out[i].cube[2] = (int32_t)r[2];
        out[i].face = (int32_t)r[3];
        out[i].t_distance = r[4];
        out[i].intersection_point[0] = r[5]; out[i].intersection_point[1] = r[6]; out[i].intersection_point[2] = r[7];
    }
    *n_out = n;
    *ended = en;
    return AIC_OK;
}

int aic_probe_powf(aic_ctx *c, const float *x, const float *y, uint32_t n, float *out) {
    if (!c || (n && (!x || !y || !out))) return fail(c, AIC_ERR_INVALID, "aic_probe_powf: bad argument");
    if (!n) return AIC_OK;
    HIP_TRY(c, hipSetDevice(c->device));
    hipError_t e = c->staging.ensure((size_t)n * 12);
    if (e != hipSuccess) return hip_fail(c, "alloc staging", e);
    float *dx = (float *)c->staging.p, *dy = dx + n, *dout = dy + n;
    HIP_TRY(c, hipMemcpyAsync(dx, x, (size_t)n * 4, hipMemcpyHostToDevice, c->stream));
    HIP_TRY(c, hipMemcpyAsync(dy, y, (size_t)n * 4, hipMemcpyHostToDevice, c->stream));
    launch_probe_powf(dx, dy, dout, n, c->stream);
    HIP_TRY(c, hipGetLastError());
    HIP_TRY(c, hipMemcpyAsync(out, dout, (size_t)n * 4, hipMemcpyDeviceToHost, c->stream));
    HIP_TRY(c, hipStreamSynchronize(c->stream));
    return AIC_OK;
}

int aic_probe_expf(aic_ctx *c, const float *x, uint32_t n, float *out) {
    if (!c || (n && (!x || !out))) return fail(c, AIC_ERR_INVALID, "aic_probe_expf: bad argument");
    if (!n) return AIC_OK;
    for (uint32_t i = 0; i < n; i++)
        if (!(std::fabs(x[i]) < 88.0f)) return fail(c, AIC_ERR_INVALID, "aic_probe_expf: x outside (-88, 88)");
    HIP_TRY(c, hipSetDevice(c->device));
    hipError_t e = c->staging.ensure((size_t)n * 8);
    if (e != hipSuccess) return hip_fail(c, "alloc staging", e);
    float *dx = (float *)c->staging.p, *dout = dx + n;
    HIP_TRY(c, hipMemcpyAsync(dx, x, (size_t)n * 4, hipMemcpyHostToDevice, c->stream));
    launch_probe_expf(dx, dout, n, c->stream);
    HIP_TRY(c, hipGetLastError());
    HIP_TRY(c, hipMemcpyAsync(out, dout, (size_t)n * 4, hipMemcpyDeviceToHost, c->stream));
    HIP_TRY(c, hipStreamSynchronize(c->stream));
    return AIC_OK;
}

int aic_probe_bloom(aic_ctx *c, uint32_t width, uint32_t height, const float *colorbuf, float exposure, const aic_options *options, uint8_t *out_rgba8,
                    uint16_t *out_mip0, uint32_t mip0_size[2]) {
    if (!c || !colorbuf || !options || !out_rgba8 || !width || !height) return fail(c, AIC_ERR_INVALID, "aic_probe_bloom: bad argument");
    if (width > 65535u || height > 65535u) return fail(c, AIC_ERR_INVALID, "aic_probe_bloom: frame dimensions above 65535 are not supported");
    if (!(exposure >= 0.f) || !(options->bloom_intensity >= 0.f)) return fail(c, AIC_ERR_INVALID, "aic_probe_bloom: exposure or bloom_intensity is negative or NaN");
    HIP_TRY(c, hipSetDevice(c->device));
    if (c->slots[0].busy) return fail(c, AIC_ERR_INVALID, "aic_probe_bloom: a submitted frame still occupies slot 0 (aic_render_wait it first)");
    const BloomGeom geom = bloom_geometry(width, height);
    const size_t npix = (size_t)width * height;
    aic_ctx::SubSlot &sb = c->slots[0].sub[0];
    hipError_t e;
    if ((e = sb.bloom_cb.ensure(npix)) != hipSuccess || (e = sb.bloom_mips.ensure(geom.texels)) != hipSuccess || (e = c->out.ensure(npix)) != hipSuccess)
        return hip_fail(c, "alloc bloom scratch", e);
    HIP_TRY(c, hipMemcpyAsync(sb.bloom_cb.p, colorbuf, npix * 16, hipMemcpyHostToDevice, c->stream));
    BloomParams bp;
    bp.colorbuf = sb.bloom_cb.p;
    bp.mips = sb.bloom_mips.p;
    bp.out = c->out.p;
    bp.exposure = exposure + 0.0f;
    bp.intensity = options->bloom_intensity;
    bp.tone_mapping = options->tone_mapping;
    bp.maximum_intensity = options->maximum_intensity;
    bp.srgb_thr = c->srgb_thr.p;
    launch_bloom(geom, bp, c->stream);
    HIP_TRY(c, hipGetLastError());
    HIP_TRY(c, hipMemcpyAsync(out_rgba8, c->out.p, npix * 4, hipMemcpyDeviceToHost, c->stream));
    if (out_mip0) HIP_TRY(c, hipMemcpyAsync(out_mip0, sb.bloom_mips.p, (size_t)geom.mw[0] * geom.mh[0] * 8, hipMemcpyDeviceToHost, c->stream));
    HIP_TRY(c, hipStreamSynchronize(c->stream));
    if (mip0_size) { mip0_size[0] = geom.mw[0]; mip0_size[1] = geom.mh[0]; }
    return AIC_OK;
}

int aic_probe_light_lut(aic_ctx *c, float out[256]) {
    if (!c || !out) return AIC_ERR_INVALID;
    HIP_TRY(c, hipSetDevice(c->device));
    HIP_TRY(c, hipMemcpy(out, c->lut.p, 256 * sizeof(float), hipMemcpyDeviceToHost));
    return AIC_OK;
}

}
```

### all_is_cubes_amd/csrc/aic_ctx.h

```cpp
#pragma once

#include <hip/hip_runtime.h>

#include <chrono>
#include <condition_variable>
#include <cstdio>
#include <mutex>
#include <string>
#include <thread>
#include <vector>

#include "../../include/aic_hip.h"
#include "aic_device.h"

namespace aic {

template <typename T>
struct DevBuf {
    T *p = nullptr;
    size_t n = 0;
    size_t cap = 0;
    hipError_t ensure(size_t count, bool keep = false, hipStream_t stream = nullptr) {
        if (count <= cap) { n = count; return hipSuccess; }
        size_t new_cap = count + count / 4 + 16;
        T *np_ = nullptr;
        hipError_t e = hipMalloc((void **)&np_, new_cap * sizeof(T));
        if (e != hipSuccess) return e;
        if (keep && p && cap) {
            e = hipMemcpyAsync(np_, p, cap * sizeof(T), hipMemcpyDeviceToDevice, stream);
            if (e == hipSuccess) e = hipStreamSynchronize(stream);
            if (e != hipSuccess) {
                (void)hipFree(np_);
                return e;
            }
        }
        if (p) (void)hipFree(p);
        p = np_;
        cap = new_cap;
        n = count;
        return hipSuccess;
    }
    void release() {
        if (p) (void)hipFree(p);
        p = nullptr;
        n = cap = 0;
    }
};

struct LightState;
void light_state_free(LightState *s);
void light_state_cubes_updated(LightState *s, uint64_t version_before, uint64_t version_after, uint32_t n, const int32_t *xyz, const uint16_t *block_index,
                               const uint8_t *light);

struct Layer {
    bool present = false;
    int32_t lo[3] = {0, 0, 0}, size[3] = {0, 0, 0};
    DevBuf<uint16_t> pool;
    DevBuf<uint32_t> cls;
    std::vector<uint32_t> host_cls;
    DevBuf<uint32_t> light;
    static constexpr int kLightSpares = 7;
    DevBuf<uint32_t> light_spare[kLightSpares];
    DevBuf<DevBlock> blocks;
    DevBuf<DevPaletteEntry> palette;
    std::vector<DevBlock> host_blocks;
    std::vector<uint32_t> vox_cap, pal_cap, vox_base, pal_base;
    uint64_t garbage_vox = 0, garbage_pal = 0;
    int32_t air_index = -1;
    int32_t sky_kind = 0;
    float sky[8][3] = {};
    uint32_t block_sky[7] = {};
    aic_options opt;
    bool opt_set = false;
    bool cls_in_code = false;
    uint64_t version = 0;
    uint64_t upload_serial = 0;
    LightState *lstate = nullptr;
    size_t n_cubes() const { return (size_t)size[0] * (size_t)size[1] * (size_t)size[2]; }
    void release() {
        pool.release(); cls.release(); light.release(); blocks.release(); palette.release();
        for (auto &sp : light_spare) sp.release();
        host_blocks.clear(); host_cls.clear(); vox_cap.clear(); pal_cap.clear(); vox_base.clear(); pal_base.clear();
        garbage_vox = garbage_pal = 0;
        present = false;
        version++;
        light_state_free(lstate);
        lstate = nullptr;
    }
};

}

using namespace aic;

struct aic_ctx {
    int device = 0;
    hipStream_t stream = nullptr;
    hipStream_t upload_stream = nullptr;
    Layer layers[2];
    DevBuf<float> lut;
    DevBuf<float> srgb_thr;
    DevBuf<uint32_t> out;
    DevBuf<DevAux> aux;
    DevBuf<unsigned char> staging;
    DevBuf<DevOrthoView> ortho_views;
    uint64_t aux_records = 0;
    bool streaming_submit = false;
    struct SubSlot {
        DevBuf<DevCounters> counters;
        DevCounters *host_counters = nullptr;
        bool counters_clean = false;
        size_t cost_clean_n = 0;
        bool record_ready = false;
        uint32_t order_key[6] = {0, 0, 0, 0, 0, 0};
        DevBuf<float4> acc;
        DevBuf<uint32_t> tile_cost, tile_order, queue_start;
        DevBuf<float4> bloom_cb;
        DevBuf<uint2> bloom_mips;
        uint32_t cost_sig[4] = {0, 0, 0, 0};
        double cost_cam[16] = {0};
        void release() {
            counters.release(); acc.release(); tile_cost.release(); tile_order.release(); queue_start.release(); bloom_cb.release(); bloom_mips.release();
            if (host_counters) (void)hipHostFree(host_counters);
            host_counters = nullptr;
            counters_clean = record_ready = false; cost_clean_n = 0;
        }
    };
    struct FrameSlot {
        hipStream_t stream = nullptr;
        hipEvent_t ev0 = nullptr, ev1 = nullptr;
        hipEvent_t ev2 = nullptr;
        SubSlot sub[kMaxSub];
        uint32_t n_sub = 1;
        bool static_ready = false;
        uint32_t static_key[6] = {0, 0, 0, 0, 0, 0};
        DevBuf<uint32_t> tile_static, queue_static;
        DevBuf<uint4> ray_cold;
        DevBuf<double> edges;
        uint32_t edges_w = 0, edges_h = 0;
        bool busy = false;
        bool diag = false;
        uint32_t variant = 0, tile_queues = 0;
        const void *light_used[2] = {nullptr, nullptr};
        uint32_t flaws = 0, local_rows = 0;
        size_t npix = 0;
        std::chrono::steady_clock::time_point t_begin;
    } slots[AIC_MAX_IN_FLIGHT];
    std::string err;
    std::FILE *dump = nullptr;
    char devname[256] = {0};
    uint32_t n_cus = 256;
    struct LightJob {
        std::thread worker;
        std::mutex mu;
        std::condition_variable cv;
        bool has_work = false, quit = false;
        bool running = false;
        bool pending = false;
        bool result_ready = false;
        int layer = 0, spare = -1;
        aic_light_params params;
        std::vector<int32_t> queue_cubes, queue_priorities;
        int rc = AIC_OK;
        aic_light_info info;
        std::string err;
    } ljob;
    struct Switches {
        int tile = 0, macro = 0;
        bool feedback = true;
        bool wait_whole_stream = false;
        uint32_t tiles_per_wave = 0;
        std::string wave_prof;
    } sw;
};

namespace aic {

extern thread_local std::string *tl_err_sink;
int fail(aic_ctx *c, int code, const char *what, hipError_t e = hipSuccess);
int hip_fail(aic_ctx *c, const char *what, hipError_t e);
#define HIP_TRY(ctx, expr)                                    \
    do {                                                      \
        hipError_t e_ = (expr);                               \
        if (e_ != hipSuccess) return hip_fail(ctx, #expr, e_); \
    } while (0)

inline bool valid_layer(int l) { return l == AIC_LAYER_WORLD || l == AIC_LAYER_UI; }

int take_light_spare(aic_ctx *c, Layer &l, int layer, size_t n, int *index);
int quiesce(aic_ctx *c);
int light_job_finish(aic_ctx *c);

}
```

### all_is_cubes_amd/csrc/aic_device.h

```cpp
#pragma once

#include <hip/hip_runtime.h>
#include <stdint.h>

namespace aic {

struct DevBlock {
    float color[4];
    float emission[3];
    uint32_t kind;
    uint32_t vlo_packed;
    uint32_t vsize_packed;
    uint32_t vox_off;
    uint32_t pal_off;
    uint32_t n_invisible;
    uint32_t pad[3];
};
static_assert(sizeof(DevBlock) == 64, "DevBlock is one 64-byte line");

struct DevPaletteEntry {
    float color[4];
    float emission[3];
    float pad;
};
static_assert(sizeof(DevPaletteEntry) == 32, "palette entry is 32 B");

struct DevOptions {
    int32_t fog;
    int32_t transparency;
    float threshold;
    int32_t lighting;
    int32_t antialiasing;
    int32_t debug_pixel_cost;
    int32_t tone_mapping;
    float maximum_intensity;
    int32_t bounce_samples;
    int32_t pad_;
    double view_distance;
};

struct DevLayer {
    const uint16_t *pool;
    const uint32_t *cls;
    const uint32_t *light;
    const DevBlock *blocks;
    const DevPaletteEntry *palette;
    int32_t lo[3];
    int32_t size[3];
    uint32_t n_blocks;
    int32_t present;
    int32_t air_index;
    int32_t sky_kind;
    float sky[8][3];
    uint32_t block_sky[7];
    DevOptions opt;
    double inv[16];
    float exposure;
    uint32_t cls_in_code;
};

static constexpr uint32_t kCubeClassShift = 14u;
static constexpr uint32_t kCubeIndexMask = (1u << kCubeClassShift) - 1u;

constexpr uint32_t kMaxTileQueues = 8;

struct DevCounters {
    unsigned long long cubes_traced;
    unsigned long long n_outer;
    unsigned long long n_inner;
    unsigned long long n_hits;
    unsigned long long n_light;
    unsigned long long bailed;
    unsigned long long prof[48];
    uint32_t tile_next;
    uint32_t waves_done;
    uint32_t tile_next_q[kMaxTileQueues][16];
#ifdef AIC_PROFILE
    uint32_t wave_prof[2048][4];
#endif
};

struct DevAux {
    int32_t hit;
    int32_t cube[3];
    int32_t voxel[3];
    int32_t resolution;
    int32_t face;
    int32_t block_index;
    uint32_t cubes_traced;
    uint32_t layer;
    double t_distance;
};

struct DevOrthoView {
    uint32_t x0, y0, w, h;
    double m[16];
    double dir[3];
};

struct DevSub {
    double inv[16];
    float backdrop[4];
    float exposure;
    int32_t has_backdrop;
    uint32_t *out;
    float4 *acc_buf;
    DevCounters *counters;
    unsigned long long *host_counters;
    const uint32_t *tile_order;
    uint32_t *tile_cost;
    const uint32_t *queue_start;
};
constexpr uint32_t kMaxSub = 8;

struct DevFrame {
    DevLayer layer;
    int32_t layer_transparency, layer_lighting;
    uint32_t width, height;
    int32_t antialias;
    float maximum_intensity;
    int32_t tone_mapping;
    uint32_t strip_rows, n_parts, part;
    uint32_t local_rows;
    uint32_t tiles_x, tiles_y;
    uint32_t tile;
    uint32_t macro;
    uint32_t macros_x, macros_y;
    uint32_t n_cus;
    uint32_t tiles_per_wave;
    int32_t pass;
    uint32_t hit_layer;
    int32_t use_init;
    int32_t pixel_centers;
    int32_t out_mode;
    const DevOrthoView *ortho;
    int32_t ortho_n;
    const double *patches;
    uint32_t n_patches;
    int32_t bare_trace;
    const double *rays;
    DevAux *aux;
    uint32_t n_queues;
    uint32_t n_sub;
    DevSub sub[kMaxSub];
    const float *light_lut;
    const float *srgb_thr;
    const double *edge_x, *edge_y;
    uint4 *ray_cold;
    uint32_t ray_cold_groups;
    uint32_t ray_mode;
    uint32_t exchange;
};

struct OrderJobs {
    const uint32_t *cost[kMaxSub];
    uint32_t *order[kMaxSub];
    uint32_t *queue_start[kMaxSub];
    uint32_t *clear_words[kMaxSub];
};

constexpr int kTile = 16;
constexpr int kClsWords = 4096;

}
```

### all_is_cubes_amd/csrc/aic_trace.hip

```cpp

#include <hip/hip_runtime.h>
#include <stdint.h>

#include <cstddef>
#include <cstdlib>

#include "aic_device.h"
#include "aic_encode.h"
#include "aic_lightmath.h"

namespace aic {

#define AIC_DEV __device__ __forceinline__

constexpr int FACE_WITHIN = 0;
constexpr int I32_MIN_ = (-2147483647 - 1);
constexpr int I32_MAX_ = 2147483647;

constexpr uint32_t FL_BEGINNING = 0, FL_INBOUNDS = 1, FL_ENDED = 2;


AIC_DEV int signum_101(double x) {
    if (x == 0.0) return 0;
    if (x != x) return 0;
// ... 731 lines not shown
    double tx, ty, tz, last_t;
    int cx, cy, cz;
    uint32_t lax;
    bool got, inbounds;
};
AIC_DEV FirstCube lvl_first_masks(const Lvl s0, const RayDir rd, int lox, int loy, int loz, int hix, int hiy, int hiz) {
    typedef unsigned long long mask_t;
    FirstCube f;
    f.tx = s0.tx; f.ty = s0.ty; f.tz = s0.tz; f.last_t = s0.last_t;
    f.cx = s0.cx; f.cy = s0.cy; f.cz = s0.cz;
    f.lax = 8u | (uint32_t)FACE_WITHIN;
    const mask_t negx = __builtin_amdgcn_ballot_w64(rd.sx < 0), posx = __builtin_amdgcn_ballot_w64(rd.sx > 0);
    const mask_t negy = __builtin_amdgcn_ballot_w64(rd.sy < 0), posy = __builtin_amdgcn_ballot_w64(rd.sy > 0);
    const mask_t negz = __builtin_amdgcn_ballot_w64(rd.sz < 0), posz = __builtin_amdgcn_ballot_w64(rd.sz > 0);
    mask_t active = __builtin_amdgcn_ballot_w64(lvl_fl(s0) != FL_ENDED);
    mask_t m_got = 0ull, m_inb = 0ull, m_stepped = 0ull;
    const uint32_t finite_classes = 0x1f8u;
    while (active != 0ull) {
        const mask_t lowx = __builtin_amdgcn_ballot_w64(f.cx < lox), highx = __builtin_amdgcn_ballot_w64(f.cx >= hix);
        const mask_t lowy = __builtin_amdgcn_ballot_w64(f.cy < loy), highy = __builtin_amdgcn_ballot_w64(f.cy >= hiy);
        const mask_t lowz = __builtin_amdgcn_ballot_w64(f.cz < loz), highz = __builtin_amdgcn_ballot_w64(f.cz >= hiz);
        const mask_t enter = (lowx & ~negx) | (highx & ~posx) | (lowy & ~negy) | (highy & ~posy) | (lowz & ~negz) | (highz & ~posz);
        const mask_t exit_ = (lowx & ~posx) | (highx & ~negx) | (lowy & ~posy) | (highy & ~negy) | (lowz & ~posz) | (highz & ~negz);
        const mask_t m_in = active & ~(enter | exit_), m_go = active & enter & ~exit_;
        const mask_t m_any = m_in | m_go;
        mask_t m_fin, sv, mx, m_stp;
        double mn;
        asm volatile(
            "s_and_saveexec_b64 %[sv], %[any]\n\t"
            "v_min_f64 %[mn], %[tx], %[ty]\n\t"
            "v_min_f64 %[mn], %[mn], %[tz]\n\t"
            "v_cmp_class_f64 %[fin], %[mn], %[cls]\n\t"
            "s_and_b64 %[stp], %[fin], %[go]\n\t"
            "s_mov_b64 exec, %[stp]\n\t"
            "v_mov_b64 %[lt], %[mn]\n\t"
            "v_cmp_eq_f64 %[mx], %[tz], %[mn]\n\t"
            "v_cmp_eq_f64 vcc, %[ty], %[mn]\n\t"
            "s_andn2_b64 vcc, vcc, %[mx]\n\t"
            "s_mov_b64 exec, %[mx]\n\t"
            "v_add_f64 %[tz], %[tz], %[tdz]\n\t"
            "v_add_u32 %[cz], %[cz], %[sz]\n\t"
            "v_mov_b32 %[lax], 2\n\t"
            "s_or_b64 %[mx], %[mx], vcc\n\t"
            "s_mov_b64 exec, vcc\n\t"
            "v_add_f64 %[ty], %[ty], %[tdy]\n\t"
            "v_add_u32 %[cy], %[cy], %[sy]\n\t"
            "v_mov_b32 %[lax], 1\n\t"
            "s_andn2_b64 exec, %[stp], %[mx]\n\t"
            "v_add_f64 %[tx], %[tx], %[tdx]\n\t"
            "v_add_u32 %[cx], %[cx], %[sx]\n\t"
            "v_mov_b32 %[lax], 0\n\t"
            "s_mov_b64 exec, %[sv]\n\t"
            : [tx] "+v"(f.tx), [ty] "+v"(f.ty), [tz] "+v"(f.tz), [lt] "+v"(f.last_t), [cx] "+v"(f.cx), [cy] "+v"(f.cy), [cz] "+v"(f.cz), [lax] "+v"(f.lax),
              [mn] "=&v"(mn), [sv] "=&s"(sv), [mx] "=&s"(mx), [fin] "=&s"(m_fin), [stp] "=&s"(m_stp)
            : [tdx] "v"(rd.tdx), [tdy] "v"(rd.tdy), [tdz] "v"(rd.tdz), [sx] "v"(rd.sx), [sy] "v"(rd.sy), [sz] "v"(rd.sz), [any] "s"(m_any), [go] "s"(m_go),
              [cls] "s"(finite_classes)
            : "vcc", "scc");
        m_got |= m_in & (m_fin | ~m_stepped);
        m_inb |= m_in & m_fin;
        m_stepped |= m_stp;
        active = m_stp;
    }
    f.got = __builtin_amdgcn_inverse_ballot_w64(m_got);
    f.inbounds = __builtin_amdgcn_inverse_ballot_w64(m_inb);
    return f;
}


template <bool VOL, int LMODE, bool DIAG, bool BIG, bool XC>
__global__ __launch_bounds__((AIC_EXCHANGE && XC && !DIAG && LMODE != 3) ? AIC_XWG_THREADS : AIC_WG_THREADS, (DIAG || LMODE == 3) ? 2 : AIC_MIN_WAVES) void trace_image_kernel(const DevFrame F) {
    constexpr bool XCHG = AIC_EXCHANGE && XC && !DIAG && LMODE != 3;
    constexpr uint32_t WGT = XCHG ? (uint32_t)AIC_XWG_THREADS : (uint32_t)AIC_WG_THREADS;
    constexpr uint32_t NPOOL = XCHG ? (uint32_t)AIC_POOL : 0u;
    constexpr uint32_t NCOL = WGT + NPOOL;
    static_assert(NPOOL <= 192u, "three tags per lane are scanned");
    const uint32_t lane = threadIdx.x & 63u;
    uint32_t tile_x0 = 0, tile_y0 = 0;
    __shared__ float s_lut[256];
    __shared__ float s_thr[kSrgbWindowWords];
    __shared__ double s_pow[64];
    pow_tables_to_lds(s_pow, threadIdx.x, WGT);
    for (uint32_t i = threadIdx.x; i < 256u; i += WGT) s_lut[i] = F.light_lut[i];
    srgb_window_to_lds(s_thr, F.srgb_thr, threadIdx.x, WGT);
    __syncthreads();
    const float *lut = s_lut;
    const int ostx = 2 * F.layer.size[1] * F.layer.size[2], osty = 2 * F.layer.size[2];
    const uint32_t hit_layer_s = F.hit_layer;
    unsigned long long pool_bits = (unsigned long long)F.layer.pool;
    asm volatile("s_mov_b64 %0, %1" : "=s"(pool_bits) : "s"(pool_bits));
    const uint32_t idx_mask = BIG ? 0xffffu : kCubeIndexMask;
    const uint32_t outer_thr = BIG ? 0x10000u : (1u << kCubeClassShift);

    double tx = 0, ty = 0, tz = 0, last_t = 0;
    double tdx = 0, tdy = 0, tdz = 0;
    uint32_t rx = 0, ry = 0, rz = 0;
    uint32_t boff = 0;
    int ssx = 0, ssy = 0, ssz = 0;
    uint32_t thr = outer_thr;
    uint32_t raw = 0;
    uint32_t lax = 8u;
    uint32_t st = 0u;
    uint32_t count = 0;
    ColorBuf acc;
    acc.l0 = acc.l1 = acc.l2 = 0.f; acc.t = 1.0f;
    float pend0 = 0.f, pend1 = 0.f, pend2 = 0.f, pend_tr = 1.f;
    uint32_t blk_pal_off = 0, blk_geo = 0, blk_vsz = 0;
    BounceRng brng{0ull, 0ull, 0ull, 0ull};
    uint32_t sec_steps = 0;
    enum { C_STX, C_STY, C_STZ,
           C_TABS,
           C_DX, C_DY, C_DZ,
           C_OX, C_OY, C_OZ, N_C64_ALL };
    enum { K_SRX, K_SRY, K_SRZ, K_SBOFF,
           K_TVIEW, K_PXY,
           K_BLK, K_S0, K_S1, K_S2, K_ST, N_C32_ALL };
    constexpr int N_C64 = XCHG ? (int)C_OX : (int)N_C64_ALL, N_C32 = XCHG ? (int)K_BLK : (int)N_C32_ALL;
    __shared__ double c64[N_C64][NCOL];
    __shared__ uint32_t c32[N_C32][NCOL];
    __shared__ uint32_t s_steps[WGT];
    __shared__ u32x4 s_pool[NPOOL ? NPOOL : 1u][10];
    constexpr uint32_t NTAG = NPOOL > 128u ? 192u : (NPOOL > 64u ? 128u : 64u);
    __shared__ uint32_t s_tag[NTAG];
    __shared__ u32x4 s_census;
    __shared__ uint8_t s_pick[WGT / 64u][2][64];
    const uint32_t tid = threadIdx.x;
    uint32_t col = tid;
    s_steps[tid] = 0u;
    if (!XCHG) c32[XCHG ? 0 : (int)K_BLK][tid] = 0u;
    c32[K_PXY][tid] = 0u;
    if (XCHG) {
        for (uint32_t i = tid; i < NTAG; i += WGT) s_tag[i] = i < NPOOL ? TAG_FREE : TAG_BUSY;
        for (uint32_t i = tid; i < NPOOL; i += WGT) {
            s_pool[i][9] = u32x4{0u, 0u, WGT + i, 0u};
            c32[K_PXY][WGT + i] = 0u;
        }
        if (tid == 0u) s_census = u32x4{0u, 0u, 0u, 0u};
        __syncthreads();
    }
    uint32_t dry = 0u;
    __shared__ uint32_t s_queues_tried[WGT / 64u];
    __shared__ uint32_t s_tile_state[WGT / 64u][4];
    __shared__ uint32_t s_idle_spins[WGT / 64u];
    if (lane == 0u) { s_queues_tried[threadIdx.x >> 6] = 0u; s_idle_spins[threadIdx.x >> 6] = 0u; }
    SurfDiag pend_d;
    double pend_t = 0.0;
    bool pend_visible = false;
    if (DIAG) {
        pend_d.nlight = 0; pend_d.res = pend_d.face = pend_d.block = 0;
        for (int a = 0; a < 3; a++) pend_d.cube[a] = pend_d.voxel[a] = 0;
    }
    uint32_t px_steps = 0, px_steps_prev = 0;
    Diag dg;
    if (DIAG) {
        dg.n_outer = dg.n_inner = dg.n_hits = dg.n_light = 0; dg.layer = 0; dg.hit = 0; dg.res = dg.face = dg.block = 0; dg.t = 0.0;
        for (int a = 0; a < 3; a++) dg.cube[a] = dg.voxel[a] = 0;
    }
    uint32_t tot_outer = 0, tot_inner = 0, tot_hits = 0, tot_light = 0;

    uint32_t ev = EV_NEWRAY | EV_TAKE;
#ifdef AIC_PROFILE
    __shared__ uint32_t s_prof[WGT / 64u][40];
    __shared__ uint32_t s_ray_t0[NCOL];
    uint32_t ray_dur_max = 0u, ray_dur_steps = 0u;
    uint32_t tail_trips = 0u, tail_events = 0u, tail_lanes = 0u;
    uint32_t *const prof = s_prof[tid >> 6];
    if (lane < 40u) prof[lane] = 0u;
// ... 1261 lines not shown
            t_enter |= m_enter;
            t_fin |= m_fin;
            t_deadpark |= (m_defer & ~m_fin) | (m_newdead & m_fin);
            m_act &= ~(m_shade | m_enter | m_fin);
            m_dead = m_newdead & m_act;
            m_fresh = 0ull;
        }
        ev = AIC_LANE(m_st) ? 0u : ev;
        ev = AIC_LANE(t_shade) ? EV_SHADE : ev;
        ev = AIC_LANE(t_enter) ? EV_ENTER : ev;
        ev = AIC_LANE(t_fin) ? EV_FINISH : ev;
        if ((t_deadpark | m_dead) != 0ull) ev = AIC_LANE(t_deadpark | m_dead) ? (ev | EV_DEAD) : ev;
#undef AIC_LANE
        }
        AIC_TICK(12);
    }

    AIC_SECTION(epilogue);
    typedef const __attribute__((address_space(4))) DevFrame KFrameE;
    typedef const __attribute__((address_space(4))) DevSub KSubE;
    KFrameE *Fe = (KFrameE *)__builtin_amdgcn_kernarg_segment_ptr();
    asm volatile("" : "+s"(Fe));
    const uint32_t n_sub_e = Fe->n_sub > 1u ? Fe->n_sub : 1u;
    KSubE &SE = Fe->sub[blockIdx.x & (n_sub_e - 1u)];
    DevCounters *const counters_e = SE.counters;
#ifdef AIC_PROFILE
    if (lane == 0) {
        prof[3] = (uint32_t)__builtin_readcyclecounter() - prof_t0;
        const uint32_t wid = blockIdx.x * (WGT / 64u) + (threadIdx.x >> 6);
        if (wid < 2048u) {
            counters_e->wave_prof[wid][0] = prof_t0;
            counters_e->wave_prof[wid][1] = prof_t0 + prof[2];
            counters_e->wave_prof[wid][2] = prof_t0 + prof[3];
            counters_e->wave_prof[wid][3] = prof[9];
        }
        atomicMax(&counters_e->prof[0], (unsigned long long)prof[3]);
        atomicMax(&counters_e->prof[1], (unsigned long long)prof[2]);
    }
#ifdef AIC_TAIL_PROF
    {
        const uint32_t wid = blockIdx.x * (WGT / 64u) + (threadIdx.x >> 6);
        const uint32_t ml = tail_trips ? (tail_lanes * 16u) / tail_trips : 0u;
        if (lane == 0 && wid < 2048u) counters_e->wave_prof[wid][3] = (tail_trips > 4095u ? 4095u : tail_trips) | ((tail_events > 1023u ? 1023u : tail_events) << 12) | ((ml > 1023u ? 1023u : ml) << 22);
    }
#endif
#ifdef AIC_RAY_PROF
    {
        uint32_t best_ = (ray_dur_max & ~1023u) | (ray_dur_steps > 1023u ? 1023u : ray_dur_steps);
#pragma unroll
        for (int off = 32; off > 0; off >>= 1) { const uint32_t o_ = (uint32_t)__shfl_down((int)best_, off, 64); best_ = o_ > best_ ? o_ : best_; }
        const uint32_t wid = blockIdx.x * (WGT / 64u) + (threadIdx.x >> 6);
        if (lane == 0 && wid < 2048u) counters_e->wave_prof[wid][3] = best_;
    }
#endif
    if (lane == 0) for (int i = 2; i < 40; i++) atomicAdd(&counters_e->prof[i], (unsigned long long)prof[i]);
#endif
    uint32_t t_end = threadIdx.x;
    asm volatile("" : "+v"(t_end));
    unsigned long long s = s_steps[t_end];
#pragma unroll
    for (int off = 32; off > 0; off >>= 1) s += __shfl_down(s, off, 64);
    if (lane == 0 && s) atomicAdd(&counters_e->cubes_traced, s);
    if (DIAG) {
        unsigned long long v[4] = {tot_outer, tot_inner, tot_hits, tot_light};
#pragma unroll
        for (int k = 0; k < 4; k++) {
#pragma unroll
            for (int off = 32; off > 0; off >>= 1) v[k] += __shfl_down(v[k], off, 64);
        }
        if (lane == 0) {
            if (v[0]) atomicAdd(&counters_e->n_outer, v[0]);
            if (v[1]) atomicAdd(&counters_e->n_inner, v[1]);
            if (v[2]) atomicAdd(&counters_e->n_hits, v[2]);
            if (v[3]) atomicAdd(&counters_e->n_light, v[3]);
        }
    }
    unsigned long long *const host_counters_e = SE.host_counters;
    if (lane == 0 && host_counters_e) {
        asm volatile("s_waitcnt vmcnt(0)" ::: "memory");
        if (atomicAdd(&counters_e->waves_done, 1u) == (gridDim.x / n_sub_e) * (blockDim.x >> 6) - 1u) {
            unsigned long long *const src = &counters_e->cubes_traced;
#pragma unroll
            for (int i = 0; i < 6; i++) host_counters_e[i] = __hip_atomic_load(&src[i], __ATOMIC_RELAXED, __HIP_MEMORY_SCOPE_AGENT);
        }
    }
}


__global__ void scatter_cubes_kernel(uint16_t *grid, uint32_t *light, const int32_t *xyz, const uint16_t *bi,
                                     const uint32_t *lt, uint32_t n, int lx, int ly, int lz, int sx, int sy, int sz,
                                     const uint32_t *cls) {
    uint32_t i = blockIdx.x * blockDim.x + threadIdx.x;
    if (i >= n) return;
    uint32_t dx = (uint32_t)xyz[3 * i + 0] - (uint32_t)lx;
    uint32_t dy = (uint32_t)xyz[3 * i + 1] - (uint32_t)ly;
    uint32_t dz = (uint32_t)xyz[3 * i + 2] - (uint32_t)lz;
    if ((dx >= (uint32_t)sx) | (dy >= (uint32_t)sy) | (dz >= (uint32_t)sz)) return;
    size_t idx = ((size_t)dx * sy + dy) * sz + dz;
    if (bi) {
        uint32_t b = bi[i];
        if (cls) b |= ((cls[b >> 4] >> ((b & 15u) << 1)) & 3u) << kCubeClassShift;
        grid[idx] = (uint16_t)b;
    }
    if (lt) light[idx] = lt[i];
}

__global__ void tag_cubes_kernel(uint16_t *grid, size_t n, const uint32_t *cls, int from_tagged, int to_tagged) {
    size_t i = (size_t)blockIdx.x * blockDim.x + threadIdx.x;
    if (i >= n) return;
    uint32_t b = grid[i];
    if (from_tagged) b &= kCubeIndexMask;
    if (to_tagged) b |= ((cls[b >> 4] >> ((b & 15u) << 1)) & 3u) << kCubeClassShift;
    grid[i] = (uint16_t)b;
}

__device__ __forceinline__ uint32_t tile_queue_of(uint32_t mt, uint32_t macros_x, uint32_t sb_shift, uint32_t n_queues) {
    uint32_t my = (uint32_t)((float)mt * __builtin_amdgcn_rcpf((float)macros_x));
    if (my * macros_x > mt) my--;
    else if ((my + 1u) * macros_x <= mt) my++;
    const uint32_t mx = mt - my * macros_x;
    const uint32_t v = (mx >> sb_shift) + 3u * (my >> sb_shift);
    return (n_queues & (n_queues - 1u)) == 0u ? (v & (n_queues - 1u)) : v % n_queues;
}
constexpr uint32_t kOrderThreads = 256;
__global__ __launch_bounds__(kOrderThreads) void order_tiles_kernel(const OrderJobs jobs, uint32_t n_tiles, uint32_t macros_x, uint32_t sb_shift, uint32_t n_queues,
                                                                    uint32_t clear_the_cost, uint32_t n_clear_words) {
    const uint32_t *__restrict__ const cost = jobs.cost[blockIdx.x];
    uint32_t *__restrict__ const order = jobs.order[blockIdx.x];
    uint32_t *__restrict__ const queue_start = jobs.queue_start[blockIdx.x];
    uint32_t *const clear_cost = (clear_the_cost && cost) ? const_cast<uint32_t *>(cost) : nullptr;
    uint32_t *const clear_words = jobs.clear_words[blockIdx.x];
    __shared__ uint32_t hist[kMaxTileQueues * 1024];
    __shared__ uint32_t scan[kOrderThreads];
    if (clear_words) for (uint32_t i = threadIdx.x; i < n_clear_words; i += kOrderThreads) clear_words[i] = 0u;
    const uint32_t tid = threadIdx.x;
    const uint32_t n_bins = n_queues * 1024u;
    const uint32_t per_thread = n_bins / kOrderThreads;
    const uint32_t *const cp = cost ? cost : order;
    const uint32_t use = cost ? ~0u : 0u;
    for (uint32_t b = tid; b < n_bins; b += kOrderThreads) hist[b] = 0;
    __syncthreads();
    for (uint32_t base = tid; base < n_tiles; base += 8u * kOrderThreads) {
        uint32_t c[8];
#pragma unroll
        for (uint32_t k = 0; k < 8u; k++) c[k] = cp[min(base + k * kOrderThreads, n_tiles - 1u)] & use;
#pragma unroll
        for (uint32_t k = 0; k < 8u; k++) {
            const uint32_t t = base + k * kOrderThreads;
            if (t < n_tiles) atomicAdd(&hist[tile_queue_of(t, macros_x, sb_shift, n_queues) * 1024u + 1023u - (c[k] < 1023u ? c[k] : 1023u)], 1u);
        }
    }
    __syncthreads();
    uint32_t mine = 0;
    for (uint32_t k = 0; k < per_thread; k++) mine += hist[tid * per_thread + k];
    scan[tid] = mine;
    __syncthreads();
    for (uint32_t off = 1; off < kOrderThreads; off <<= 1) {
        const uint32_t v = tid >= off ? scan[tid - off] : 0u;
        __syncthreads();
        scan[tid] += v;
        __syncthreads();
    }
    uint32_t run = scan[tid] - mine;
    for (uint32_t k = 0; k < per_thread; k++) {
        const uint32_t h = hist[tid * per_thread + k];
        hist[tid * per_thread + k] = run;
        run += h;
    }
// ... 14 lines not shown
            }
        }
    }
}

__global__ void assemble_strips_kernel(const uint32_t *gathered, uint32_t *out, uint32_t w, uint32_t h, uint32_t strip_rows,
                                       uint32_t n_parts, uint32_t max_rows) {
    size_t i = (size_t)blockIdx.x * blockDim.x + threadIdx.x;
    if (i >= (size_t)w * h) return;
    uint32_t y = (uint32_t)(i / w), x = (uint32_t)(i % w);
    uint32_t strip = y / strip_rows;
    uint32_t part = strip % n_parts;
    uint32_t lrow = (strip / n_parts) * strip_rows + (y % strip_rows);
    out[i] = gathered[((size_t)part * max_rows + lrow) * w + x];
}

__global__ void probe_raycast_kernel(const double *od, int use_bounds, const int *lohi, int include_exit, uint32_t max_steps,
                                     double *out_rec, uint32_t *n_out, int *ended) {
    if (threadIdx.x != 0 || blockIdx.x != 0) return;
    const double ox = od[0], oy = od[1], oz = od[2], dx = od[3], dy = od[4], dz = od[5];
    int lo[3] = {lohi[0], lohi[1], lohi[2]}, hi[3] = {lohi[3], lohi[4], lohi[5]};
    if (!use_bounds) {
        lo[0] = lo[1] = lo[2] = I32_MIN_ + 1;
        hi[0] = hi[1] = hi[2] = I32_MAX_ - 1;
    }
    const RayDir rd = raydir_init(dx, dy, dz);
    const LvlLim ll = lvl_init(ox, oy, oz, rd, use_bounds != 0, lo[0], lo[1], lo[2], hi[0], hi[1], hi[2], include_exit != 0,
                               0.5 / sqrt(rd.dx * rd.dx + rd.dy * rd.dy + rd.dz * rd.dz));
    Lvl s = ll.s;
    const Lim lim = ll.lim;
    uint32_t n = 0;
    *ended = 0;
    bool first_by_masks = use_bounds != 0 && include_exit != 0;
    while (n < max_steps) {
        NextResult nr;
        if (first_by_masks) {
            first_by_masks = false;
            const FirstCube f = lvl_first_masks(s, rd, lo[0], lo[1], lo[2], hi[0], hi[1], hi[2]);
            nr.got = f.got; nr.is_exit = false;
            nr.s.tx = f.tx; nr.s.ty = f.ty; nr.s.tz = f.tz; nr.s.last_t = f.last_t;
            nr.s.cx = f.cx; nr.s.cy = f.cy; nr.s.cz = f.cz;
            const uint32_t face = (f.lax & 8u) ? (f.lax & 7u) : (((f.lax == 0u ? rd.sx : (f.lax == 1u ? rd.sy : rd.sz)) > 0 ? 1u : 4u) + f.lax);
            nr.s.st = (face << 2) | 256u | (f.inbounds ? (FL_INBOUNDS | ((uint32_t)pick_axis(f.tx, f.ty, f.tz) << 5) | 128u) : FL_ENDED);
        } else {
            nr = lvl_next(s, lim, rd, lo[0], lo[1], lo[2], hi[0], hi[1], hi[2]);
        }
        s = nr.s;
        if (!nr.got) {
            *ended = 1;
            break;
        }
        double ip[3];
        intersection_point(s, ox, oy, oz, dx, dy, dz, ip);
        double *r = out_rec + 8 * (size_t)n;
        r[0] = (double)s.cx; r[1] = (double)s.cy; r[2] = (double)s.cz;
        r[3] = (double)lvl_face(s); r[4] = s.last_t; r[5] = ip[0]; r[6] = ip[1]; r[7] = ip[2];
        n++;
    }
    *n_out = n;
}

AIC_DEV float powf_exact(float x, float y) { return (float)pow((double)x, (double)y); }

__global__ void probe_powf_kernel(const float *x, const float *y, float *out, uint32_t n) {
    __shared__ double s_pow[64];
    pow_tables_to_lds(s_pow, threadIdx.x, blockDim.x);
    __syncthreads();
    const uint32_t i = blockIdx.x * blockDim.x + threadIdx.x;
    if (i >= n) return;
    out[i] = powf_table_domain(x[i], y[i]) ? powf_table(x[i], y[i], s_pow) : powf_exact(x[i], y[i]);
}

__global__ void probe_expf_kernel(const float *x, float *out, uint32_t n) {
    __shared__ double s_pow[64];
    pow_tables_to_lds(s_pow, threadIdx.x, blockDim.x);
    __syncthreads();
    const uint32_t i = blockIdx.x * blockDim.x + threadIdx.x;
    if (i >= n) return;
    out[i] = expf_table(x[i], s_pow);
}


template <bool VOL, int LMODE, bool DIAG, bool BIG, bool XC>
static void launch_trace_x(const DevFrame &F, hipStream_t stream) {
    const uint32_t n_tiles = F.tiles_x * F.tiles_y;
    constexpr bool XCHG = AIC_EXCHANGE && XC && !DIAG && LMODE != 3;
    constexpr uint32_t WGT = XCHG ? (uint32_t)AIC_XWG_THREADS : (uint32_t)AIC_WG_THREADS;
    const uint32_t wg_waves = WGT / 64u;
    const uint32_t n_sub = F.n_sub > 1u ? F.n_sub : 1u;
    const uint32_t resident_groups = F.n_cus * 4u * (uint32_t)((DIAG || LMODE == 3) ? 2 : AIC_MIN_WAVES) / wg_waves / n_sub;
    const uint32_t tiles_per_wave = F.tiles_per_wave ? F.tiles_per_wave : 1u;
    const uint32_t by_tiles = (n_tiles + wg_waves - 1u) / wg_waves;
    uint32_t grid = (n_tiles + wg_waves * tiles_per_wave - 1u) / (wg_waves * tiles_per_wave);
    const uint32_t floor_groups = by_tiles < 128u ? by_tiles : 128u;
    if (grid < floor_groups) grid = floor_groups;
    if (grid > resident_groups) grid = resident_groups;
    if (XCHG && F.antialias && grid > F.ray_cold_groups / n_sub) grid = F.ray_cold_groups / n_sub;
    grid *= n_sub;
    if (grid == 0) return;
    DevFrame G = F;
    G.ray_mode = (F.layer.present && !F.pixel_centers && !F.patches && !F.rays && !F.ortho_n && F.edge_x && F.edge_y) ? (F.n_parts > 1u ? 1u : 0u) : 2u;
    hipLaunchKernelGGL((trace_image_kernel<VOL, LMODE, DIAG, BIG, XC>), dim3(grid), dim3(WGT), 0, stream, G);
}

template <bool VOL, int LMODE, bool DIAG, bool BIG>
static void launch_trace(const DevFrame &F, hipStream_t stream) {
    if constexpr (AIC_EXCHANGE && !DIAG && LMODE != 3) {
        if (F.exchange && (F.ray_cold || !F.antialias)) { launch_trace_x<VOL, LMODE, DIAG, BIG, true>(F, stream); return; }
    }
    launch_trace_x<VOL, LMODE, DIAG, BIG, false>(F, stream);
}

template <bool DIAG, bool BIG>
static void launch_trace_diag(const DevFrame &F, bool vol, int lmode, hipStream_t stream) {
    if (vol) {
        if (lmode == 0) launch_trace<true, 0, DIAG, BIG>(F, stream);
        else if (lmode == 1) launch_trace<true, 1, DIAG, BIG>(F, stream);
        else if (lmode == 3) launch_trace<true, 3, DIAG, BIG>(F, stream);
        else launch_trace<true, 2, DIAG, BIG>(F, stream);
    } else {
        if (lmode == 0) launch_trace<false, 0, DIAG, BIG>(F, stream);
        else if (lmode == 1) launch_trace<false, 1, DIAG, BIG>(F, stream);
        else if (lmode == 3) launch_trace<false, 3, DIAG, BIG>(F, stream);
        else launch_trace<false, 2, DIAG, BIG>(F, stream);
    }
}

size_t trace_ray_cold_bytes(uint32_t n_cus, uint32_t *groups) {
    if (!AIC_EXCHANGE) { *groups = 0; return 0; }
    const uint32_t g = n_cus * 4u * (uint32_t)AIC_MIN_WAVES / ((uint32_t)AIC_XWG_THREADS / 64u);
    *groups = g;
    return (size_t)g * ((size_t)AIC_XWG_THREADS + (size_t)AIC_POOL) * 16u;
}

void launch_trace_image(const DevFrame &F, bool diag, hipStream_t stream) {
    const bool vol = F.layer_transparency == 1;
    const int l = F.layer_lighting;
    const int lmode = l == 0 ? 0 : (l == 1 ? 1 : (l == 5 ? 3 : 2));
    const bool big = F.layer.cls_in_code == 0u;
    if (diag) {
        if (big) launch_trace_diag<true, true>(F, vol, lmode, stream);
        else launch_trace_diag<true, false>(F, vol, lmode, stream);
    } else {
        if (big) launch_trace_diag<false, true>(F, vol, lmode, stream);
        else launch_trace_diag<false, false>(F, vol, lmode, stream);
    }
}

void launch_tag_cubes(uint16_t *grid, size_t n, const uint32_t *cls, int from_tagged, int to_tagged, hipStream_t stream) {
    if (!n) return;
    hipLaunchKernelGGL(tag_cubes_kernel, dim3((unsigned)((n + 255) / 256)), dim3(256), 0, stream, grid, n, cls, from_tagged, to_tagged);
}

void launch_scatter_cubes(uint16_t *grid, uint32_t *light, const int32_t *xyz, const uint16_t *bi, const uint32_t *lt,
                          uint32_t n, const int lo[3], const int size[3], const uint32_t *cls, hipStream_t stream) {
    if (!n) return;
    hipLaunchKernelGGL(scatter_cubes_kernel, dim3((n + 255) / 256), dim3(256), 0, stream, grid, light, xyz, bi, lt, n, lo[0],
                       lo[1], lo[2], size[0], size[1], size[2], cls);
}

void launch_probe_powf(const float *x, const float *y, float *out, uint32_t n, hipStream_t stream) {
    if (!n) return;
    hipLaunchKernelGGL(probe_powf_kernel, dim3((n + 255u) / 256u), dim3(256), 0, stream, x, y, out, n);
}

void launch_probe_expf(const float *x, float *out, uint32_t n, hipStream_t stream) {
    if (!n) return;
    hipLaunchKernelGGL(probe_expf_kernel, dim3((n + 255u) / 256u), dim3(256), 0, stream, x, out, n);
}

void launch_order_tiles_jobs(const OrderJobs &jobs, uint32_t n_jobs, uint32_t n_tiles, uint32_t macros_x, uint32_t sb_shift, uint32_t n_queues, hipStream_t stream,
                             bool clear_cost, uint32_t n_clear_words) {
    if (!n_tiles || !n_jobs) return;
    if (n_queues < 1u) n_queues = 1u;
    if (n_queues > kMaxTileQueues) n_queues = kMaxTileQueues;
    hipLaunchKernelGGL(order_tiles_kernel, dim3(n_jobs), dim3(kOrderThreads), 0, stream, jobs, n_tiles, macros_x ? macros_x : 1u, sb_shift, n_queues, clear_cost ? 1u : 0u,
                       n_clear_words);
}
void launch_order_tiles(const uint32_t *cost, uint32_t *order, uint32_t n_tiles, uint32_t macros_x, uint32_t sb_shift, uint32_t n_queues, uint32_t *queue_start,
                        hipStream_t stream, bool clear_cost, uint32_t *clear_words, uint32_t n_clear_words) {
    OrderJobs jobs{};
    jobs.cost[0] = cost; jobs.order[0] = order; jobs.queue_start[0] = queue_start; jobs.clear_words[0] = clear_words;
    launch_order_tiles_jobs(jobs, 1u, n_tiles, macros_x, sb_shift, n_queues, stream, clear_cost, n_clear_words);
}

void launch_assemble_strips(const uint32_t *gathered, uint32_t *out, uint32_t w, uint32_t h, uint32_t strip_rows,
                            uint32_t n_parts, uint32_t max_rows, hipStream_t stream) {
    size_t n = (size_t)w * h;
    if (!n) return;
    hipLaunchKernelGGL(assemble_strips_kernel, dim3((unsigned)((n + 255) / 256)), dim3(256), 0, stream, gathered, out, w, h,
                       strip_rows, n_parts, max_rows);
}

void launch_probe_raycast(const double *od, int use_bounds, const int *lohi, int include_exit, uint32_t max_steps,
                          double *out_rec, uint32_t *n_out, int *ended, hipStream_t stream) {
    hipLaunchKernelGGL(probe_raycast_kernel, dim3(1), dim3(64), 0, stream, od, use_bounds, lohi, include_exit, max_steps, out_rec,
                       n_out, ended);
}

}
```

### include/aic_hip.h

```cpp
#ifndef AIC_HIP_H
#define AIC_HIP_H

#include <stdint.h>

#ifdef __cplusplus
extern "C" {
#endif

#define AIC_ABI_VERSION 3

#define AIC_OK 0
#define AIC_ERR_INVALID 1
#define AIC_ERR_NO_DEVICE 2
#define AIC_ERR_OOM 3
#define AIC_ERR_DEVICE 4
#define AIC_ERR_UNSUPPORTED 5

#define AIC_LAYER_WORLD 0
#define AIC_LAYER_UI 1

#define AIC_FLAW_UNSUPPORTED 1u
#define AIC_FLAW_NO_BLOOM 2u

#define AIC_BLOCK_ONE 1u
// ... 106 lines not shown
} aic_pixel_aux;

typedef struct aic_ctx aic_ctx;

aic_ctx *aic_create(int device_id, int *status);
void aic_destroy(aic_ctx *ctx);
const char *aic_last_error(const aic_ctx *ctx);
int aic_abi_version(void);
int aic_device_name(const aic_ctx *ctx, char *buf, uint32_t buf_len);

int aic_upload_space(aic_ctx *ctx, int layer, const aic_space_desc *space);
int aic_clear_space(aic_ctx *ctx, int layer);
int aic_update_cubes(aic_ctx *ctx, int layer, uint32_t n, const int32_t *xyz, const uint16_t *block_index,
                     const uint8_t *light);
int aic_update_light_volume(aic_ctx *ctx, int layer, const uint8_t *light);
int aic_replace_block(aic_ctx *ctx, int layer, uint32_t index, const aic_block_desc *desc, const uint16_t *voxels,
                      const float *palette);
int aic_replace_blocks(aic_ctx *ctx, int layer, uint32_t n, const uint32_t *indices, const aic_block_desc *descs,
                       const uint16_t *const *voxels, const float *const *palettes);
int aic_compact(aic_ctx *ctx, int layer);
int aic_set_options(aic_ctx *ctx, int layer, const aic_options *options);

int aic_render(aic_ctx *ctx, const aic_frame_desc *frame, void *out_rgba8, int out_is_device, aic_frame_info *info);
#define AIC_MAX_IN_FLIGHT 32u
int aic_render_submit(aic_ctx *ctx, const aic_frame_desc *frame, void *out_device, uint32_t slot);
int aic_render_wait(aic_ctx *ctx, uint32_t slot, aic_frame_info *info);
int aic_render_submit_batch(aic_ctx *ctx, uint32_t n_frames, const aic_frame_desc *frames, void *const *out_devices, uint32_t slot);
int aic_render_wait_batch(aic_ctx *ctx, uint32_t slot, uint32_t n_frames, aic_frame_info *infos);
int aic_trace_patches(aic_ctx *ctx, const aic_frame_desc *frame, uint32_t n, const double *rects, void *out_rgba8,
                      aic_pixel_aux *aux, aic_frame_info *info);
#define AIC_RAYS_NO_SKY 128u
#define AIC_RAYS_DEVICE 256u
int aic_trace_rays(aic_ctx *ctx, int layer, uint32_t n, const double *rays, uint32_t flags, float exposure, void *out, aic_pixel_aux *aux,
                   aic_frame_info *info);
uint32_t aic_partition_rows(uint32_t height, const aic_partition *partition);
int aic_assemble_strips(aic_ctx *ctx, const void *gathered_device, void *out_device, uint32_t width, uint32_t height,
                        uint32_t strip_rows, uint32_t n_parts);
int aic_assemble_strips_async(aic_ctx *ctx, const void *gathered_device, void *out_device, uint32_t width, uint32_t height,
                              uint32_t strip_rows, uint32_t n_parts);
int aic_assemble_strips_on(aic_ctx *ctx, const void *gathered_device, void *out_device, uint32_t width, uint32_t height,
                           uint32_t strip_rows, uint32_t n_parts, void *hip_stream);
int aic_read_aux(aic_ctx *ctx, aic_pixel_aux *out, uint64_t n_records);
int aic_synchronize(aic_ctx *ctx);
void *aic_stream(aic_ctx *ctx);
int aic_wait_event(aic_ctx *ctx, void *hip_event);
int aic_stream_wait_frame(aic_ctx *ctx, uint32_t slot, void *hip_stream);

int aic_ortho_image_size(const int32_t lo[3], const int32_t size[3], int resolution, uint32_t *width, uint32_t *height);
int aic_render_orthographic(aic_ctx *ctx, int layer, int resolution, void *out_rgba8, int out_is_device, uint32_t *width,
                            uint32_t *height, aic_frame_info *info);

typedef struct aic_multi aic_multi;
aic_multi *aic_create_multi(int n_devices, const int *device_ids, int *status);
void aic_destroy_multi(aic_multi *m);
int aic_multi_device_count(const aic_multi *m);
aic_ctx *aic_multi_context(aic_multi *m, int i);
const char *aic_multi_last_error(const aic_multi *m);
int aic_multi_upload_space(aic_multi *m, int layer, const aic_space_desc *space);
int aic_multi_clear_space(aic_multi *m, int layer);
int aic_multi_update_cubes(aic_multi *m, int layer, uint32_t n, const int32_t *xyz, const uint16_t *block_index, const uint8_t *light);
int aic_multi_update_light_volume(aic_multi *m, int layer, const uint8_t *light);
int aic_multi_replace_blocks(aic_multi *m, int layer, uint32_t n, const uint32_t *indices, const aic_block_desc *descs,
                             const uint16_t *const *voxels, const float *const *palettes);
int aic_multi_set_options(aic_multi *m, int layer, const aic_options *options);
int aic_multi_render(aic_multi *m, const aic_frame_desc *frame, void *out_rgba8, int out_is_device, aic_frame_info *info);
#define AIC_MULTI_MAX_IN_FLIGHT 8u
int aic_multi_render_submit(aic_multi *m, const aic_frame_desc *frame, void *out_rgba8, int out_is_device, uint32_t slot);
int aic_multi_render_wait(aic_multi *m, uint32_t slot, aic_frame_info *info);

typedef struct aic_rc_step {
    int32_t cube[3];
    int32_t face;
    double t_distance;
    double intersection_point[3];
} aic_rc_step;
int aic_probe_raycast(aic_ctx *ctx, const double origin[3], const double direction[3], int use_bounds,
                      const int32_t lo[3], const int32_t hi[3], int include_exit, uint32_t max_steps,
                      aic_rc_step *out, uint32_t *n_out, int *ended);
int aic_probe_powf(aic_ctx *ctx, const float *x, const float *y, uint32_t n, float *out);
int aic_probe_expf(aic_ctx *ctx, const float *x, uint32_t n, float *out);
int aic_probe_bloom(aic_ctx *ctx, uint32_t width, uint32_t height, const float *colorbuf, float exposure, const aic_options *options,
                    uint8_t *out_rgba8, uint16_t *out_mip0, uint32_t mip0_size[2]);
int aic_probe_light_lut(aic_ctx *ctx, float out[256]);

typedef struct aic_light_params {
    int32_t maximum_distance;
    int32_t fast;
    int32_t epsilon;
    int32_t batch;
    int32_t queue_order;
    int32_t n_queue;
    int32_t lanes_per_cube;
    int32_t hooks;
    const int32_t *queue_cubes;
    const int32_t *queue_priorities;
    uint64_t max_updates;
} aic_light_params;
#define AIC_LIGHT_HOOK_SESSION 1
#define AIC_LIGHT_HOOK_POOL_SHIFT 8
typedef struct aic_light_info {
    uint64_t updates;
    uint64_t batches;
    uint64_t cost;
    double device_ms;
    double total_ms;
    uint32_t queue_left;
    uint32_t pad;
    uint64_t bundles_visited;
} aic_light_info;
int aic_evaluate_light(aic_ctx *ctx, int layer, const aic_light_params *params, aic_light_info *info);
int aic_evaluate_light_submit(aic_ctx *ctx, int layer, const aic_light_params *params);
int aic_evaluate_light_wait(aic_ctx *ctx, int layer, aic_light_info *info);
int aic_evaluate_light_poll(aic_ctx *ctx, int layer, int *done);
int aic_light_cubes_changed(aic_ctx *ctx, int layer, uint32_t n, const int32_t *xyz, int queue_order);
int aic_read_light_volume(aic_ctx *ctx, int layer, uint8_t *out);
int aic_read_light_cubes(aic_ctx *ctx, int layer, uint32_t n, const int32_t *xyz, uint8_t *out);
uint32_t aic_light_chart(float *weights, uint32_t *children, uint32_t *depth);
int aic_probe_derived(aic_ctx *ctx, int layer, float *out, uint8_t *out_opaque);
int aic_probe_log2f(aic_ctx *ctx, const float *x, uint32_t n, float *out);
int aic_multi_evaluate_light(aic_multi *m, int layer, const aic_light_params *params, aic_light_info *info);
int aic_multi_light_cubes_changed(aic_multi *m, int layer, uint32_t n, const int32_t *xyz, int queue_order);

#ifdef __cplusplus
}
#endif
#endif
```

### rust/all-is-cubes-hip/src/ffi.rs

```rust
#![allow(non_camel_case_types, missing_docs, clippy::missing_safety_doc)]

use core::ffi::{c_char, c_int, c_void};

pub const AIC_ABI_VERSION: c_int = 3;
pub const AIC_OK: c_int = 0;
pub const AIC_ERR_INVALID: c_int = 1;
pub const AIC_ERR_NO_DEVICE: c_int = 2;
pub const AIC_ERR_OOM: c_int = 3;
pub const AIC_ERR_DEVICE: c_int = 4;
pub const AIC_ERR_UNSUPPORTED: c_int = 5;
pub const AIC_LAYER_WORLD: c_int = 0;
pub const AIC_LAYER_UI: c_int = 1;
pub const AIC_BLOCK_ONE: u32 = 1;
pub const AIC_BLOCK_AIR: u32 = 2;
pub const AIC_FLAW_UNSUPPORTED: u32 = 1;
pub const AIC_FLAW_NO_BLOOM: u32 = 2;
pub const AIC_FRAME_COUNTERS: u32 = 1;
pub const AIC_FRAME_AUX: u32 = 2;
pub const AIC_FRAME_PIXEL_CENTERS: u32 = 4;
pub const AIC_FRAME_OUT_LINEAR: u32 = 8;
pub const AIC_FRAME_OUT_COLORBUF: u32 = 16;
pub const AIC_FRAME_NO_FEEDBACK: u32 = 32;
pub const AIC_FRAME_BLOOM: u32 = 64;
pub const AIC_RAYS_NO_SKY: u32 = 128;
// ... 44 lines not shown
#[repr(C)]
#[derive(Clone, Copy, Debug)]
pub struct aic_options {
    pub fog: i32,
    pub transparency: i32,
    pub threshold: f32,
    pub lighting: i32,
    pub bounce_samples: i32,
    pub antialiasing: i32,
    pub debug_pixel_cost: i32,
    pub tone_mapping: i32,
    pub maximum_intensity: f32,
    pub bloom_intensity: f32,
    pub view_distance: f64,
}

#[repr(C)]
#[derive(Clone, Copy, Debug)]
pub struct aic_camera {
    pub inverse_projection_view: [f64; 16],
    pub exposure: f32,
    pub reserved: i32,
}

#[repr(C)]
#[derive(Clone, Copy, Debug, Default)]
pub struct aic_partition {
    pub strip_rows: u32,
    pub n_parts: u32,
    pub part: u32,
    pub reserved: u32,
}

#[repr(C)]
#[derive(Clone, Copy, Debug)]
pub struct aic_frame_desc {
    pub width: u32,
    pub height: u32,
    pub world: aic_camera,
    pub ui: aic_camera,
    pub backdrop: [f32; 4],
    pub partition: aic_partition,
    pub flags: u32,
    pub tuning: u32,
}

#[repr(C)]
#[derive(Clone, Copy, Debug, Default)]
pub struct aic_frame_info {
    pub cubes_traced: u64,
    pub n_outer: u64,
    pub n_inner: u64,
    pub n_hits: u64,
    pub n_light: u64,
    pub kernel_ms: f32,
    pub total_ms: f32,
    pub rows_rendered: u32,
    pub flaws: u32,
    pub variant: u32,
    pub tile_queues: u32,
}

#[repr(C)]
#[derive(Clone, Copy, Debug, Default)]
pub struct aic_pixel_aux {
    pub hit: i32,
    pub cube: [i32; 3],
    pub voxel: [i32; 3],
    pub resolution: i32,
    pub face: i32,
    pub block_index: i32,
    pub cubes_traced: u32,
    pub layer: u32,
    pub t_distance: f64,
}

#[repr(C)]
#[derive(Clone, Copy, Debug, Default)]
pub struct aic_rc_step {
    pub cube: [i32; 3],
    pub face: i32,
    pub t_distance: f64,
    pub intersection_point: [f64; 3],
}

#[repr(C)]
pub struct aic_ctx {
    _private: [u8; 0],
}
#[repr(C)]
pub struct aic_multi {
    _private: [u8; 0],
}

#[repr(C)]
#[derive(Clone, Copy, Debug)]
pub struct aic_light_params {
    pub maximum_distance: i32,
    pub fast: i32,
    pub epsilon: i32,
    pub batch: i32,
    pub queue_order: i32,
    pub n_queue: i32,
    pub lanes_per_cube: i32,
    pub hooks: i32,
    pub queue_cubes: *const i32,
    pub queue_priorities: *const i32,
    pub max_updates: u64,
}

#[repr(C)]
#[derive(Clone, Copy, Debug, Default)]
pub struct aic_light_info {
    pub updates: u64,
    pub batches: u64,
    pub cost: u64,
    pub device_ms: f64,
    pub total_ms: f64,
    pub queue_left: u32,
    pub pad: u32,
    pub bundles_visited: u64,
}

unsafe extern "C" {
    pub fn aic_create(device_id: c_int, status: *mut c_int) -> *mut aic_ctx;
    pub fn aic_destroy(ctx: *mut aic_ctx);
    pub fn aic_last_error(ctx: *const aic_ctx) -> *const c_char;
    pub fn aic_abi_version() -> c_int;
    pub fn aic_device_name(ctx: *const aic_ctx, buf: *mut c_char, buf_len: u32) -> c_int;
    pub fn aic_upload_space(ctx: *mut aic_ctx, layer: c_int, space: *const aic_space_desc) -> c_int;
    pub fn aic_clear_space(ctx: *mut aic_ctx, layer: c_int) -> c_int;
    pub fn aic_update_cubes(ctx: *mut aic_ctx, layer: c_int, n: u32, xyz: *const i32, block_index: *const u16, light: *const u8) -> c_int;
    pub fn aic_update_light_volume(ctx: *mut aic_ctx, layer: c_int, light: *const u8) -> c_int;
    pub fn aic_replace_block(ctx: *mut aic_ctx, layer: c_int, index: u32, desc: *const aic_block_desc, voxels: *const u16, palette: *const f32) -> c_int;
    pub fn aic_replace_blocks(ctx: *mut aic_ctx, layer: c_int, n: u32, indices: *const u32, descs: *const aic_block_desc, voxels: *const *const u16, palettes: *const *const f32) -> c_int;
    pub fn aic_compact(ctx: *mut aic_ctx, layer: c_int) -> c_int;
    pub fn aic_set_options(ctx: *mut aic_ctx, layer: c_int, options: *const aic_options) -> c_int;
    pub fn aic_render(ctx: *mut aic_ctx, frame: *const aic_frame_desc, out_rgba8: *mut c_void, out_is_device: c_int, info: *mut aic_frame_info) -> c_int;
    pub fn aic_render_submit(ctx: *mut aic_ctx, frame: *const aic_frame_desc, out_device: *mut c_void, slot: u32) -> c_int;
    pub fn aic_render_wait(ctx: *mut aic_ctx, slot: u32, info: *mut aic_frame_info) -> c_int;
    pub fn aic_render_submit_batch(ctx: *mut aic_ctx, n_frames: u32, frames: *const aic_frame_desc, out_devices: *const *mut c_void, slot: u32) -> c_int;
    pub fn aic_render_wait_batch(ctx: *mut aic_ctx, slot: u32, n_frames: u32, infos: *mut aic_frame_info) -> c_int;
    pub fn aic_trace_patches(ctx: *mut aic_ctx, frame: *const aic_frame_desc, n: u32, rects: *const f64, out_rgba8: *mut c_void, aux: *mut aic_pixel_aux, info: *mut aic_frame_info) -> c_int;
    pub fn aic_partition_rows(height: u32, partition: *const aic_partition) -> u32;
    pub fn aic_assemble_strips(ctx: *mut aic_ctx, gathered_device: *const c_void, out_device: *mut c_void, width: u32, height: u32, strip_rows: u32, n_parts: u32) -> c_int;
    pub fn aic_assemble_strips_async(ctx: *mut aic_ctx, gathered_device: *const c_void, out_device: *mut c_void, width: u32, height: u32, strip_rows: u32, n_parts: u32) -> c_int;
    pub fn aic_assemble_strips_on(ctx: *mut aic_ctx, gathered_device: *const c_void, out_device: *mut c_void, width: u32, height: u32, strip_rows: u32, n_parts: u32, hip_stream: *mut c_void) -> c_int;
    pub fn aic_trace_rays(ctx: *mut aic_ctx, layer: c_int, n: u32, rays: *const f64, flags: u32, exposure: f32, out: *mut c_void, aux: *mut aic_pixel_aux, info: *mut aic_frame_info) -> c_int;
    pub fn aic_read_aux(ctx: *mut aic_ctx, out: *mut aic_pixel_aux, n_records: u64) -> c_int;
    pub fn aic_synchronize(ctx: *mut aic_ctx) -> c_int;
    pub fn aic_stream(ctx: *mut aic_ctx) -> *mut c_void;
    pub fn aic_wait_event(ctx: *mut aic_ctx, hip_event: *mut c_void) -> c_int;
    pub fn aic_stream_wait_frame(ctx: *mut aic_ctx, slot: u32, hip_stream: *mut c_void) -> c_int;
    pub fn aic_ortho_image_size(lo: *const i32, size: *const i32, resolution: c_int, width: *mut u32, height: *mut u32) -> c_int;
    pub fn aic_render_orthographic(ctx: *mut aic_ctx, layer: c_int, resolution: c_int, out_rgba8: *mut c_void, out_is_device: c_int, width: *mut u32, height: *mut u32, info: *mut aic_frame_info) -> c_int;
    pub fn aic_create_multi(n_devices: c_int, device_ids: *const c_int, status: *mut c_int) -> *mut aic_multi;
    pub fn aic_destroy_multi(m: *mut aic_multi);
    pub fn aic_multi_device_count(m: *const aic_multi) -> c_int;
    pub fn aic_multi_context(m: *mut aic_multi, i: c_int) -> *mut aic_ctx;
    pub fn aic_multi_last_error(m: *const aic_multi) -> *const c_char;
    pub fn aic_multi_upload_space(m: *mut aic_multi, layer: c_int, space: *const aic_space_desc) -> c_int;
    pub fn aic_multi_clear_space(m: *mut aic_multi, layer: c_int) -> c_int;
    pub fn aic_multi_update_cubes(m: *mut aic_multi, layer: c_int, n: u32, xyz: *const i32, block_index: *const u16, light: *const u8) -> c_int;
    pub fn aic_multi_update_light_volume(m: *mut aic_multi, layer: c_int, light: *const u8) -> c_int;
    pub fn aic_multi_replace_blocks(m: *mut aic_multi, layer: c_int, n: u32, indices: *const u32, descs: *const aic_block_desc, voxels: *const *const u16, palettes: *const *const f32) -> c_int;
    pub fn aic_multi_set_options(m: *mut aic_multi, layer: c_int, options: *const aic_options) -> c_int;
    pub fn aic_multi_render(m: *mut aic_multi, frame: *const aic_frame_desc, out_rgba8: *mut c_void, out_is_device: c_int, info: *mut aic_frame_info) -> c_int;
    pub fn aic_multi_render_submit(m: *mut aic_multi, frame: *const aic_frame_desc, out_rgba8: *mut c_void, out_is_device: c_int, slot: u32) -> c_int;
    pub fn aic_multi_render_wait(m: *mut aic_multi, slot: u32, info: *mut aic_frame_info) -> c_int;
    pub fn aic_probe_raycast(ctx: *mut aic_ctx, origin: *const f64, direction: *const f64, use_bounds: c_int, lo: *const i32, hi: *const i32, include_exit: c_int, max_steps: u32, out: *mut aic_rc_step, n_out: *mut u32, ended: *mut c_int) -> c_int;
    pub fn aic_probe_powf(ctx: *mut aic_ctx, x: *const f32, y: *const f32, n: u32, out: *mut f32) -> c_int;
    pub fn aic_probe_expf(ctx: *mut aic_ctx, x: *const f32, n: u32, out: *mut f32) -> c_int;
    pub fn aic_probe_bloom(ctx: *mut aic_ctx, width: u32, height: u32, colorbuf: *const f32, exposure: f32, options: *const aic_options, out_rgba8: *mut u8, out_mip0: *mut u16, mip0_size: *mut u32) -> c_int;
    pub fn aic_probe_light_lut(ctx: *mut aic_ctx, out: *mut f32) -> c_int;
    pub fn aic_evaluate_light(ctx: *mut aic_ctx, layer: c_int, params: *const aic_light_params, info: *mut aic_light_info) -> c_int;
    pub fn aic_evaluate_light_submit(ctx: *mut aic_ctx, layer: c_int, params: *const aic_light_params) -> c_int;
    pub fn aic_evaluate_light_wait(ctx: *mut aic_ctx, layer: c_int, info: *mut aic_light_info) -> c_int;
    pub fn aic_evaluate_light_poll(ctx: *mut aic_ctx, layer: c_int, done: *mut c_int) -> c_int;
    pub fn aic_light_cubes_changed(ctx: *mut aic_ctx, layer: c_int, n: u32, xyz: *const i32, queue_order: c_int) -> c_int;
    pub fn aic_read_light_volume(ctx: *mut aic_ctx, layer: c_int, out: *mut u8) -> c_int;
    pub fn aic_read_light_cubes(ctx: *mut aic_ctx, layer: c_int, n: u32, xyz: *const i32, out: *mut u8) -> c_int;
    pub fn aic_light_chart(weights: *mut f32, children: *mut u32, depth: *mut u32) -> u32;
    pub fn aic_probe_derived(ctx: *mut aic_ctx, layer: c_int, out: *mut f32, out_opaque: *mut u8) -> c_int;
    pub fn aic_probe_log2f(ctx: *mut aic_ctx, x: *const f32, n: u32, out: *mut f32) -> c_int;
    pub fn aic_multi_evaluate_light(m: *mut aic_multi, layer: c_int, params: *const aic_light_params, info: *mut aic_light_info) -> c_int;
    pub fn aic_multi_light_cubes_changed(m: *mut aic_multi, layer: c_int, n: u32, xyz: *const i32, queue_order: c_int) -> c_int;
}
```

Baseline: 6244.

## Estimate concurrent frame residency from device timestamps to size tiles per wave

The trace kernel now stamps start and end wall-clock ticks into the frame counters. A host-side Residency model uses these to learn which in-flight frame slots actually overlap on the GPU and groups slots that never overlap into shared classes. When sizing tiles per wave, the submit path now uses the number of truly co-resident frame classes instead of simply counting busy slots. An optional env knob lets slots share streams. The change adds an atomic and a timestamp per workgroup plus event queries per submit, and it risks misjudging overlap and choosing a worse tiling.

```diff
diff --git a/all_is_cubes_amd/abi.py b/all_is_cubes_amd/abi.py
--- a/all_is_cubes_amd/abi.py
+++ b/all_is_cubes_amd/abi.py
@@ -45,7 +45,7 @@
     "aic_abi_version", "aic_create", "aic_destroy", "aic_last_error", "aic_device_name", "aic_upload_space",
     "aic_clear_space", "aic_update_cubes", "aic_update_light_volume", "aic_replace_block", "aic_replace_blocks", "aic_compact", "aic_set_options",
     "aic_render", "aic_render_submit", "aic_render_wait", "aic_render_submit_batch", "aic_render_wait_batch", "aic_trace_patches", "aic_trace_rays", "aic_partition_rows", "aic_assemble_strips", "aic_assemble_strips_async", "aic_assemble_strips_on", "aic_read_aux", "aic_synchronize", "aic_stream", "aic_wait_event", "aic_stream_wait_frame",
-    "aic_probe_raycast", "aic_probe_light_lut", "aic_probe_powf", "aic_probe_expf", "aic_probe_bloom",
+    "aic_probe_raycast", "aic_probe_light_lut", "aic_probe_powf", "aic_probe_expf", "aic_probe_bloom", "aic_probe_slot_residency", "aic_model_slot_residency",
     "aic_ortho_image_size", "aic_render_orthographic",
     "aic_evaluate_light", "aic_evaluate_light_submit", "aic_evaluate_light_wait", "aic_evaluate_light_poll", "aic_light_cubes_changed", "aic_read_light_volume", "aic_read_light_cubes", "aic_light_chart", "aic_probe_derived", "aic_probe_log2f",
     "aic_create_multi", "aic_destroy_multi", "aic_multi_device_count", "aic_multi_context", "aic_multi_last_error", "aic_multi_upload_space",
@@ -120,6 +120,31 @@
     _fields_ = [("cubes_traced", C.c_uint64), ("n_outer", C.c_uint64), ("n_inner", C.c_uint64), ("n_hits", C.c_uint64),
                 ("n_light", C.c_uint64), ("kernel_ms", C.c_float), ("total_ms", C.c_float), ("rows_rendered", C.c_uint32),
                 ("flaws", C.c_uint32), ("variant", C.c_uint32), ("tile_queues", C.c_uint32)]
+
+
+class SlotResidency(C.Structure):
+    _fields_ = [("start_ticks", C.c_uint64), ("end_ticks", C.c_uint64), ("workgroups", C.c_uint32), ("resident_workgroups", C.c_uint32),
+                ("tiles_per_wave", C.c_uint32), ("queue_class", C.c_uint32), ("classes_beside", C.c_uint32), ("reserved", C.c_uint32)]
+
+
+class ResidencyEvent(C.Structure):
+    _fields_ = [("kind", C.c_uint32), ("slot", C.c_uint32), ("running", C.c_uint32), ("reserved", C.c_uint32),
+                ("start_ticks", C.c_uint64), ("end_ticks", C.c_uint64)]
+
+
+def model_slot_residency(events):
+    lib = load()
+    ev = (ResidencyEvent * max(1, len(events)))()
+    for e, rec in zip(ev, events):
+        if rec[0] == "submit":
+            e.kind, e.slot, e.running = 0, rec[1], sum(1 << int(s) for s in rec[2])
+        else:
+            e.kind, e.slot, e.start_ticks, e.end_ticks = 1, rec[1], rec[2], rec[3]
+    out = (C.c_uint32 * max(1, len(events)))()
+    rc = lib.aic_model_slot_residency(len(events), ev, out)
+    if rc != AIC_OK:
+        raise AicError(rc, "aic_model_slot_residency")
+    return [int(out[i]) for i, rec in enumerate(events) if rec[0] == "submit"]
 
 
 PIXEL_AUX_DTYPE = np.dtype(
@@ -177,6 +202,8 @@
         lib.aic_probe_raycast.argtypes = [C.c_void_p, C.c_void_p, C.c_void_p, C.c_int, C.c_void_p, C.c_void_p, C.c_int,
                                           C.c_uint32, C.c_void_p, C.POINTER(C.c_uint32), C.POINTER(C.c_int)]
         lib.aic_probe_light_lut.argtypes = [C.c_void_p, C.c_void_p]
+        lib.aic_probe_slot_residency.argtypes = [C.c_void_p, C.c_uint32, C.POINTER(SlotResidency)]
+        lib.aic_model_slot_residency.argtypes = [C.c_uint32, C.POINTER(ResidencyEvent), C.POINTER(C.c_uint32)]
         lib.aic_probe_powf.argtypes = [C.c_void_p, C.c_void_p, C.c_void_p, C.c_uint32, C.c_void_p]
         lib.aic_probe_expf.argtypes = [C.c_void_p, C.c_void_p, C.c_uint32, C.c_void_p]
         lib.aic_probe_bloom.argtypes = [C.c_void_p, C.c_uint32, C.c_uint32, C.c_void_p, C.c_float, C.POINTER(Options), C.c_void_p, C.c_void_p,
@@ -602,6 +629,11 @@
     def probe_light_lut(self) -> np.ndarray:
         out = np.zeros(256, np.float32)
         self._check(self._lib.aic_probe_light_lut(self._h, out.ctypes.data))
+        return out
+
+    def probe_slot_residency(self, slot: int) -> SlotResidency:
+        out = SlotResidency()
+        self._check(self._lib.aic_probe_slot_residency(self._h, int(slot), C.byref(out)))
         return out
 
 
diff --git a/all_is_cubes_amd/csrc/aic_abi.cpp b/all_is_cubes_amd/csrc/aic_abi.cpp
--- a/all_is_cubes_amd/csrc/aic_abi.cpp
+++ b/all_is_cubes_amd/csrc/aic_abi.cpp
@@ -20,7 +20,7 @@
 #include "aic_device.h"
 
 namespace aic {
-void launch_trace_image(const DevFrame &F, bool diag, hipStream_t stream);
+TraceGrid launch_trace_image(const DevFrame &F, bool diag, hipStream_t stream);
 size_t trace_ray_cold_bytes(uint32_t n_cus, uint32_t *groups);
 void launch_scatter_cubes(uint16_t *grid, uint32_t *light, const int32_t *xyz, const uint16_t *bi, const uint32_t *lt,
                           uint32_t n, const int lo[3], const int size[3], const uint32_t *cls, hipStream_t stream);
@@ -42,6 +42,7 @@
 static_assert(sizeof(aic_pixel_aux) == sizeof(DevAux), "aux record layout");
 
 static_assert(sizeof(aic_block_desc) == 48, "aic_block_desc is 48 bytes");
+static_assert(kResidSlots == AIC_MAX_IN_FLIGHT, "the residency estimator keeps a bit per frame slot");
 
 namespace {
 
@@ -281,6 +282,7 @@
         c->sw.feedback = env_int("AIC_TILE_FEEDBACK", 1) != 0;
         c->sw.wait_whole_stream = env_int("AIC_WAIT_WHOLE_STREAM", 0) != 0;
         c->sw.tiles_per_wave = (uint32_t)std::max(0, env_int("AIC_TILES_PER_WAVE", 0));
+        c->sw.slot_streams = (uint32_t)std::min(std::max(0, env_int("AIC_SLOT_STREAMS", 0)), (int)AIC_MAX_IN_FLIGHT);
         if (const char *p = std::getenv("AIC_WAVE_PROF")) c->sw.wave_prof = p;
     }
     if (const char *path = std::getenv("AIC_DUMP")) {
@@ -295,7 +297,8 @@
     for (uint32_t i = 0; ok && i < 8u && i < AIC_MAX_IN_FLIGHT; i++) {
         aic_ctx::FrameSlot &fs = c->slots[i];
         if (i == 0) fs.stream = c->stream;
-        else ok = hipStreamCreateWithFlags(&fs.stream, hipStreamNonBlocking) == hipSuccess;
+        else if (c->sw.slot_streams && i >= c->sw.slot_streams) fs.stream = c->slots[i % c->sw.slot_streams].stream;
+        else ok = (fs.own_stream = hipStreamCreateWithFlags(&fs.stream, hipStreamNonBlocking) == hipSuccess);
         ok = ok && hipEventCreate(&fs.ev0) == hipSuccess && hipEventCreate(&fs.ev1) == hipSuccess && hipEventCreate(&fs.ev2) == hipSuccess && fs.sub[0].counters.ensure(1) == hipSuccess;
     }
     ok = ok && hipStreamCreateWithFlags(&c->upload_stream, hipStreamNonBlocking) == hipSuccess;
@@ -359,16 +362,17 @@
         c->ljob.worker.join();
     }
     if (c->stream) (void)hipStreamSynchronize(c->stream);
+    for (uint32_t i = 0; i < AIC_MAX_IN_FLIGHT; i++)
+        if (c->slots[i].stream) (void)hipStreamSynchronize(c->slots[i].stream);
     for (uint32_t i = 0; i < AIC_MAX_IN_FLIGHT; i++) {
         aic_ctx::FrameSlot &fs = c->slots[i];
-        if (fs.stream) (void)hipStreamSynchronize(fs.stream);
         for (auto &sb : fs.sub) sb.release();
         fs.ray_cold.release(); fs.edges.release();
         if (fs.ev0) (void)hipEventDestroy(fs.ev0);
         if (fs.ev1) (void)hipEventDestroy(fs.ev1);
         if (fs.ev2) (void)hipEventDestroy(fs.ev2);
         fs.tile_static.release(); fs.queue_static.release();
-        if (i > 0 && fs.stream) (void)hipStreamDestroy(fs.stream);
+        if (fs.own_stream) (void)hipStreamDestroy(fs.stream);
     }
     for (auto &l : c->layers) l.release();
     c->lut.release(); c->srgb_thr.release(); c->out.release(); c->aux.release(); c->staging.release(); c->ortho_views.release();
@@ -838,14 +842,28 @@
     }
     F.light_lut = c->lut.p;
     F.n_cus = c->n_cus;
+    uint32_t beside = 0;
+    fs.watched = false;
+    if (c->streaming_submit && k == 1u && npix) {
+        uint32_t running = 0;
+        for (uint32_t i = 0; i < AIC_MAX_IN_FLIGHT; i++) {
+            aic_ctx::FrameSlot &o = c->slots[i];
+            if (i == slot || !o.busy || !o.running) continue;
+            if (hipEventQuery(o.ev2) == hipSuccess) o.running = false;
+            else running |= 1u << i;
+        }
+        (void)hipGetLastError();
+        beside = c->residency.submit(slot, running);
+        fs.watched = true;
+    } else {
+        c->residency.forget(slot);
+    }
     F.tiles_per_wave = c->sw.tiles_per_wave ? c->sw.tiles_per_wave : (c->streaming_submit ? 4u : 1u);
     if (!c->sw.tiles_per_wave && c->streaming_submit && k == 1u) {
-        uint32_t busy_others = 0;
-        for (uint32_t i = 0; i < AIC_MAX_IN_FLIGHT; i++) busy_others += (i != slot && c->slots[i].busy) ? 1u : 0u;
         const uint32_t resident_waves = (uint32_t)c->n_cus * 16u;
         const uint32_t tpw_full = (F.tiles_x * F.tiles_y + resident_waves - 1u) / resident_waves;
-        if (tpw_full >= 4u && busy_others > 0u) {
-            const uint32_t t = tpw_full * (busy_others < 4u ? busy_others : 4u);
+        if (tpw_full >= 4u && beside > 0u) {
+            const uint32_t t = tpw_full * (beside < 4u ? beside : 4u);
             F.tiles_per_wave = t < 32u ? t : (tpw_full > 32u ? tpw_full : 32u);
         }
     }
@@ -1020,7 +1038,9 @@
     F.layer_lighting = hl[0].opt.lighting;
     fs.variant = diag ? AIC_VARIANT_RECORDING : ((F.exchange && hl[0].opt.lighting != 5 && (F.ray_cold || !F.antialias)) ? AIC_VARIANT_EXCHANGING : AIC_VARIANT_PLAIN);
     fs.tile_queues = F.n_queues;
-    launch_trace_image(F, diag, fs.stream);
+    fs.grid_now = launch_trace_image(F, diag, fs.stream);
+    fs.tpw_now = F.tiles_per_wave;
+    fs.beside_now = beside;
     HIP_TRY(c, hipGetLastError());
     if (bloom) {
         const BloomGeom geom = bloom_geometry(f->width, f->height);
@@ -1044,6 +1064,7 @@
 #endif
     HIP_TRY(c, hipEventRecord(fs.ev2, fs.stream));
     fs.busy = true;
+    fs.running = true;
     bool cleared = false;
     if (use_feedback && n_tiles) {
         OrderJobs jobs;
@@ -1095,10 +1116,20 @@
         fs.busy = false;
         if (whole_stream || c->sw.wait_whole_stream) HIP_TRY(c, hipStreamSynchronize(fs.stream));
         else HIP_TRY(c, hipEventSynchronize(fs.ev2));
+        fs.running = false;
         HIP_TRY(c, hipEventElapsedTime(&kernel_ms, fs.ev0, fs.ev1));
         for (uint32_t j = 0; j < k; j++) {
             DevCounters hc;
             std::memcpy(&hc, fs.sub[j].host_counters, sizeof(hc));
+            if (fs.watched) {
+                fs.watched = false;
+                if (hc.t_start && hc.t_end >= hc.t_start) {
+                    c->residency.collect(slot, hc.t_start, hc.t_end);
+                    fs.resid = aic_slot_residency{hc.t_start, hc.t_end, fs.grid_now.groups, fs.grid_now.resident, fs.tpw_now, slot, fs.beside_now, 0u};
+                } else {
+                    c->residency.forget(slot);
+                }
+            }
             if (hc.bailed) return fail(c, AIC_ERR_DEVICE, "trace kernel: a wave gave up waiting for rays in transit between waves; the frame has unwritten pixels");
             if (info) {
                 info->cubes_traced += hc.cubes_traced;
@@ -1358,8 +1389,14 @@
 static int ensure_slot(aic_ctx *c, uint32_t slot) {
     aic_ctx::FrameSlot &fs = c->slots[slot];
     if (fs.stream && fs.ev0 && fs.ev1 && fs.ev2 && fs.sub[0].counters.p) return AIC_OK;
+    if (!fs.stream && c->sw.slot_streams && slot >= c->sw.slot_streams) {
+        const uint32_t base = slot % c->sw.slot_streams;
+        { const int rs = ensure_slot(c, base); if (rs != AIC_OK) return rs; }
+        fs.stream = c->slots[base].stream;
+    }
     if (!fs.stream) {
         HIP_TRY(c, hipStreamCreateWithFlags(&fs.stream, hipStreamNonBlocking));
+        fs.own_stream = true;
         hipEvent_t ev = nullptr;
         HIP_TRY(c, hipEventCreateWithFlags(&ev, hipEventDisableTiming));
         hipError_t e1 = hipEventRecord(ev, c->stream);
@@ -1588,6 +1625,30 @@
     return AIC_OK;
 }
 
+int aic_probe_slot_residency(aic_ctx *c, uint32_t slot, aic_slot_residency *out) {
+    if (!c || !out || slot >= AIC_MAX_IN_FLIGHT) return fail(c, AIC_ERR_INVALID, "aic_probe_slot_residency: bad argument");
+    *out = c->slots[slot].resid;
+    out->queue_class = c->residency.class_of(slot);
+    return AIC_OK;
+}
+
+int aic_model_slot_residency(uint32_t n_events, const aic_residency_event *events, uint32_t *out) {
+    if (n_events && (!events || !out)) return AIC_ERR_INVALID;
+    Residency r;
+    for (uint32_t i = 0; i < n_events; i++) {
+        const aic_residency_event &e = events[i];
+        if (e.slot >= AIC_MAX_IN_FLIGHT || e.kind > 1u) return AIC_ERR_INVALID;
+        if (e.kind == 0u) {
+            const uint32_t beside = r.submit(e.slot, e.running);
+            out[i] = beside < 4u ? beside : 4u;
+        } else {
+            r.collect(e.slot, e.start_ticks, e.end_ticks);
+            out[i] = 0xffffffffu;
+        }
+    }
+    return AIC_OK;
+}
+
 int aic_probe_light_lut(aic_ctx *c, float out[256]) {
     if (!c || !out) return AIC_ERR_INVALID;
     HIP_TRY(c, hipSetDevice(c->device));
diff --git a/all_is_cubes_amd/csrc/aic_ctx.h b/all_is_cubes_amd/csrc/aic_ctx.h
--- a/all_is_cubes_amd/csrc/aic_ctx.h
+++ b/all_is_cubes_amd/csrc/aic_ctx.h
@@ -12,6 +12,7 @@
 
 #include "../../include/aic_hip.h"
 #include "aic_device.h"
+#include "aic_residency.h"
 
 namespace aic {
 
@@ -128,6 +129,7 @@
     };
     struct FrameSlot {
         hipStream_t stream = nullptr;
+        bool own_stream = false;
         hipEvent_t ev0 = nullptr, ev1 = nullptr;
         hipEvent_t ev2 = nullptr;
         SubSlot sub[kMaxSub];
@@ -139,6 +141,11 @@
         DevBuf<double> edges;
         uint32_t edges_w = 0, edges_h = 0;
         bool busy = false;
+        bool running = false;
+        bool watched = false;
+        TraceGrid grid_now = {0, 0};
+        uint32_t tpw_now = 0, beside_now = 0;
+        aic_slot_residency resid = {0, 0, 0, 0, 0, 0, 0, 0};
         bool diag = false;
         uint32_t variant = 0, tile_queues = 0;
         const void *light_used[2] = {nullptr, nullptr};
@@ -146,6 +153,7 @@
         size_t npix = 0;
         std::chrono::steady_clock::time_point t_begin;
     } slots[AIC_MAX_IN_FLIGHT];
+    Residency residency;
     std::string err;
     std::FILE *dump = nullptr;
     char devname[256] = {0};
@@ -170,6 +178,7 @@
         bool feedback = true;
         bool wait_whole_stream = false;
         uint32_t tiles_per_wave = 0;
+        uint32_t slot_streams = 0;
         std::string wave_prof;
     } sw;
 };
diff --git a/all_is_cubes_amd/csrc/aic_device.h b/all_is_cubes_amd/csrc/aic_device.h
--- a/all_is_cubes_amd/csrc/aic_device.h
+++ b/all_is_cubes_amd/csrc/aic_device.h
@@ -75,6 +75,8 @@
     uint32_t tile_next;
     uint32_t waves_done;
     uint32_t tile_next_q[kMaxTileQueues][16];
+    unsigned long long t_start, t_end;
+    uint32_t arrived, pad_arrived;
 #ifdef AIC_PROFILE
     uint32_t wave_prof[2048][4];
 #endif
@@ -152,6 +154,10 @@
     uint32_t exchange;
 };
 
+struct TraceGrid {
+    uint32_t groups, resident;
+};
+
 struct OrderJobs {
     const uint32_t *cost[kMaxSub];
     uint32_t *order[kMaxSub];
diff --git a/all_is_cubes_amd/csrc/aic_residency.h b/all_is_cubes_amd/csrc/aic_residency.h
--- /dev/null
+++ b/all_is_cubes_amd/csrc/aic_residency.h
@@ -0,0 +1,95 @@
+#pragma once
+
+#include <cstdint>
+#include <cstring>
+
+namespace aic {
+
+constexpr uint32_t kResidSlots = 32;
+constexpr uint32_t kResidHeldRounds = 2;
+
+struct Residency {
+    struct Slot {
+        uint32_t serial = 0;
+        uint32_t done_serial = 0;
+        uint64_t t0 = 0, t1 = 0;
+        uint32_t ahead[kResidSlots];
+        uint32_t done_ahead[kResidSlots];
+        Slot() { std::memset(ahead, 0, sizeof(ahead)); std::memset(done_ahead, 0, sizeof(done_ahead)); }
+    } slots[kResidSlots];
+    uint8_t distinct[kResidSlots][kResidSlots];
+    uint8_t serial_seen[kResidSlots][kResidSlots];
+    uint8_t cls[kResidSlots];
+    uint32_t next_serial = 1;
+    bool cls_stale = false;
+
+    Residency() {
+        std::memset(distinct, 0, sizeof(distinct));
+        std::memset(serial_seen, 0, sizeof(serial_seen));
+        for (uint32_t i = 0; i < kResidSlots; i++) cls[i] = (uint8_t)i;
+    }
+
+    bool held(uint32_t a, uint32_t b) const { return !distinct[a][b] && serial_seen[a][b] >= kResidHeldRounds; }
+
+    uint32_t class_of(uint32_t slot) {
+        if (cls_stale) {
+            for (uint32_t i = 0; i < kResidSlots; i++) cls[i] = (uint8_t)i;
+            for (bool moved = true; moved;) {
+                moved = false;
+                for (uint32_t a = 0; a < kResidSlots; a++)
+                    for (uint32_t b = a + 1; b < kResidSlots; b++)
+                        if (held(a, b) && cls[a] != cls[b]) {
+                            const uint8_t lo = cls[a] < cls[b] ? cls[a] : cls[b];
+                            cls[a] = cls[b] = lo;
+                            moved = true;
+                        }
+            }
+            cls_stale = false;
+        }
+        return cls[slot];
+    }
+
+    uint32_t submit(uint32_t slot, uint32_t running) {
+        Slot &s = slots[slot];
+        running &= ~(1u << slot);
+        s.serial = next_serial++;
+        if (!next_serial) next_serial = 1;
+        const uint32_t own = class_of(slot);
+        uint32_t seen = 0, n = 0;
+        for (uint32_t i = 0; i < kResidSlots; i++) {
+            const bool runs = ((running >> i) & 1u) && slots[i].serial;
+            s.ahead[i] = runs ? slots[i].serial : 0u;
+            if (!((running >> i) & 1u)) continue;
+            const uint32_t c = class_of(i);
+            if (c != own && !((seen >> c) & 1u)) { seen |= 1u << c; n++; }
+        }
+        return n;
+    }
+
+    void collect(uint32_t slot, uint64_t t0, uint64_t t1) {
+        Slot &s = slots[slot];
+        if (!s.serial) return;
+        s.done_serial = s.serial;
+        s.serial = 0;
+        s.t0 = t0;
+        s.t1 = t1;
+        std::memcpy(s.done_ahead, s.ahead, sizeof(s.ahead));
+        for (uint32_t i = 0; i < kResidSlots; i++) {
+            const Slot &o = slots[i];
+            if (i == slot || !o.done_serial) continue;
+            if (s.t0 < o.t1 && o.t0 < s.t1) {
+                if (!distinct[slot][i]) { distinct[slot][i] = distinct[i][slot] = 1; cls_stale = true; }
+                continue;
+            }
+            const bool behind = (s.done_ahead[i] == o.done_serial && s.t0 >= o.t1) || (o.done_ahead[slot] == s.done_serial && o.t0 >= s.t1);
+            if (behind && !distinct[slot][i] && serial_seen[slot][i] < 255u) {
+                serial_seen[slot][i] = serial_seen[i][slot] = (uint8_t)(serial_seen[slot][i] + 1u);
+                if (serial_seen[slot][i] == kResidHeldRounds) cls_stale = true;
+            }
+        }
+    }
+
+    void forget(uint32_t slot) { slots[slot].serial = 0; }
+};
+
+}
diff --git a/all_is_cubes_amd/csrc/aic_trace.hip b/all_is_cubes_amd/csrc/aic_trace.hip
--- a/all_is_cubes_amd/csrc/aic_trace.hip
+++ b/all_is_cubes_amd/csrc/aic_trace.hip
@@ -837,6 +837,20 @@
     pow_tables_to_lds(s_pow, threadIdx.x, WGT);
     for (uint32_t i = threadIdx.x; i < 256u; i += WGT) s_lut[i] = F.light_lut[i];
     srgb_window_to_lds(s_thr, F.srgb_thr, threadIdx.x, WGT);
+    if (threadIdx.x == 0u) {
+        typedef const __attribute__((address_space(4))) DevFrame KFrameS;
+        KFrameS *Fs = (KFrameS *)__builtin_amdgcn_kernarg_segment_ptr();
+        asm volatile("" : "+s"(Fs));
+        const uint32_t n_sub_s = Fs->n_sub > 1u ? Fs->n_sub : 1u;
+        DevCounters *const counters_s = Fs->sub[blockIdx.x & (n_sub_s - 1u)].counters;
+#ifdef AIC_PROFILE
+        const bool stamped = Fs->pass != 1;
+#else
+        const bool stamped = Fs->sub[blockIdx.x & (n_sub_s - 1u)].host_counters != nullptr;
+#endif
+        if (stamped && atomicAdd(&counters_s->arrived, 1u) == 0u)
+            __hip_atomic_store(&counters_s->t_start, (unsigned long long)wall_clock64(), __ATOMIC_RELAXED, __HIP_MEMORY_SCOPE_AGENT);
+    }
     __syncthreads();
     const float *lut = s_lut;
     const int ostx = 2 * F.layer.size[1] * F.layer.size[2], osty = 2 * F.layer.size[2];
@@ -2264,8 +2278,13 @@
             unsigned long long *const src = &counters_e->cubes_traced;
 #pragma unroll
             for (int i = 0; i < 6; i++) host_counters_e[i] = __hip_atomic_load(&src[i], __ATOMIC_RELAXED, __HIP_MEMORY_SCOPE_AGENT);
+            host_counters_e[offsetof(DevCounters, t_start) / 8u] = __hip_atomic_load(&counters_e->t_start, __ATOMIC_RELAXED, __HIP_MEMORY_SCOPE_AGENT);
+            host_counters_e[offsetof(DevCounters, t_end) / 8u] = (unsigned long long)wall_clock64();
         }
     }
+#ifdef AIC_PROFILE
+    if (lane == 0 && Fe->pass != 1) atomicMax(&counters_e->t_end, (unsigned long long)wall_clock64());
+#endif
 }
 
 
@@ -2446,7 +2465,7 @@
 
 
 template <bool VOL, int LMODE, bool DIAG, bool BIG, bool XC>
-static void launch_trace_x(const DevFrame &F, hipStream_t stream) {
+static TraceGrid launch_trace_x(const DevFrame &F, hipStream_t stream) {
     const uint32_t n_tiles = F.tiles_x * F.tiles_y;
     constexpr bool XCHG = AIC_EXCHANGE && XC && !DIAG && LMODE != 3;
     constexpr uint32_t WGT = XCHG ? (uint32_t)AIC_XWG_THREADS : (uint32_t)AIC_WG_THREADS;
@@ -2461,32 +2480,33 @@
     if (grid > resident_groups) grid = resident_groups;
     if (XCHG && F.antialias && grid > F.ray_cold_groups / n_sub) grid = F.ray_cold_groups / n_sub;
     grid *= n_sub;
-    if (grid == 0) return;
+    if (grid == 0) return TraceGrid{0u, resident_groups * n_sub};
     DevFrame G = F;
     G.ray_mode = (F.layer.present && !F.pixel_centers && !F.patches && !F.rays && !F.ortho_n && F.edge_x && F.edge_y) ? (F.n_parts > 1u ? 1u : 0u) : 2u;
     hipLaunchKernelGGL((trace_image_kernel<VOL, LMODE, DIAG, BIG, XC>), dim3(grid), dim3(WGT), 0, stream, G);
+    return TraceGrid{grid, resident_groups * n_sub};
 }
 
 template <bool VOL, int LMODE, bool DIAG, bool BIG>
-static void launch_trace(const DevFrame &F, hipStream_t stream) {
+static TraceGrid launch_trace(const DevFrame &F, hipStream_t stream) {
     if constexpr (AIC_EXCHANGE && !DIAG && LMODE != 3) {
-        if (F.exchange && (F.ray_cold || !F.antialias)) { launch_trace_x<VOL, LMODE, DIAG, BIG, true>(F, stream); return; }
-    }
-    launch_trace_x<VOL, LMODE, DIAG, BIG, false>(F, stream);
+        if (F.exchange && (F.ray_cold || !F.antialias)) return launch_trace_x<VOL, LMODE, DIAG, BIG, true>(F, stream);
+    }
+    return launch_trace_x<VOL, LMODE, DIAG, BIG, false>(F, stream);
 }
 
 template <bool DIAG, bool BIG>
-static void launch_trace_diag(const DevFrame &F, bool vol, int lmode, hipStream_t stream) {
+static TraceGrid launch_trace_diag(const DevFrame &F, bool vol, int lmode, hipStream_t stream) {
     if (vol) {
-        if (lmode == 0) launch_trace<true, 0, DIAG, BIG>(F, stream);
-        else if (lmode == 1) launch_trace<true, 1, DIAG, BIG>(F, stream);
-        else if (lmode == 3) launch_trace<true, 3, DIAG, BIG>(F, stream);
-        else launch_trace<true, 2, DIAG, BIG>(F, stream);
+        if (lmode == 0) return launch_trace<true, 0, DIAG, BIG>(F, stream);
+        if (lmode == 1) return launch_trace<true, 1, DIAG, BIG>(F, stream);
+        if (lmode == 3) return launch_trace<true, 3, DIAG, BIG>(F, stream);
+        return launch_trace<true, 2, DIAG, BIG>(F, stream);
     } else {
-        if (lmode == 0) launch_trace<false, 0, DIAG, BIG>(F, stream);
-        else if (lmode == 1) launch_trace<false, 1, DIAG, BIG>(F, stream);
-        else if (lmode == 3) launch_trace<false, 3, DIAG, BIG>(F, stream);
-        else launch_trace<false, 2, DIAG, BIG>(F, stream);
+        if (lmode == 0) return launch_trace<false, 0, DIAG, BIG>(F, stream);
+        if (lmode == 1) return launch_trace<false, 1, DIAG, BIG>(F, stream);
+        if (lmode == 3) return launch_trace<false, 3, DIAG, BIG>(F, stream);
+        return launch_trace<false, 2, DIAG, BIG>(F, stream);
     }
 }
 
@@ -2497,18 +2517,13 @@
     return (size_t)g * ((size_t)AIC_XWG_THREADS + (size_t)AIC_POOL) * 16u;
 }
 
-void launch_trace_image(const DevFrame &F, bool diag, hipStream_t stream) {
+TraceGrid launch_trace_image(const DevFrame &F, bool diag, hipStream_t stream) {
     const bool vol = F.layer_transparency == 1;
     const int l = F.layer_lighting;
     const int lmode = l == 0 ? 0 : (l == 1 ? 1 : (l == 5 ? 3 : 2));
     const bool big = F.layer.cls_in_code == 0u;
-    if (diag) {
-        if (big) launch_trace_diag<true, true>(F, vol, lmode, stream);
-        else launch_trace_diag<true, false>(F, vol, lmode, stream);
-    } else {
-        if (big) launch_trace_diag<false, true>(F, vol, lmode, stream);
-        else launch_trace_diag<false, false>(F, vol, lmode, stream);
-    }
+    if (diag) return big ? launch_trace_diag<true, true>(F, vol, lmode, stream) : launch_trace_diag<true, false>(F, vol, lmode, stream);
+    return big ? launch_trace_diag<false, true>(F, vol, lmode, stream) : launch_trace_diag<false, false>(F, vol, lmode, stream);
 }
 
 void launch_tag_cubes(uint16_t *grid, size_t n, const uint32_t *cls, int from_tagged, int to_tagged, hipStream_t stream) {
diff --git a/include/aic_hip.h b/include/aic_hip.h
--- a/include/aic_hip.h
+++ b/include/aic_hip.h
@@ -212,6 +212,21 @@
 int aic_probe_bloom(aic_ctx *ctx, uint32_t width, uint32_t height, const float *colorbuf, float exposure, const aic_options *options,
                     uint8_t *out_rgba8, uint16_t *out_mip0, uint32_t mip0_size[2]);
 int aic_probe_light_lut(aic_ctx *ctx, float out[256]);
+typedef struct aic_slot_residency {
+    uint64_t start_ticks, end_ticks;
+    uint32_t workgroups;
+    uint32_t resident_workgroups;
+    uint32_t tiles_per_wave;
+    uint32_t queue_class;
+    uint32_t classes_beside;
+    uint32_t reserved;
+} aic_slot_residency;
+int aic_probe_slot_residency(aic_ctx *ctx, uint32_t slot, aic_slot_residency *out);
+typedef struct aic_residency_event {
+    uint32_t kind, slot, running, reserved;
+    uint64_t start_ticks, end_ticks;
+} aic_residency_event;
+int aic_model_slot_residency(uint32_t n_events, const aic_residency_event *events, uint32_t *out);
 
 typedef struct aic_light_params {
     int32_t maximum_distance;
diff --git a/rust/all-is-cubes-hip/src/ffi.rs b/rust/all-is-cubes-hip/src/ffi.rs
--- a/rust/all-is-cubes-hip/src/ffi.rs
+++ b/rust/all-is-cubes-hip/src/ffi.rs
@@ -150,6 +150,30 @@
     pub face: i32,
     pub t_distance: f64,
     pub intersection_point: [f64; 3],
+}
+
+#[repr(C)]
+#[derive(Clone, Copy, Debug, Default)]
+pub struct aic_slot_residency {
+    pub start_ticks: u64,
+    pub end_ticks: u64,
+    pub workgroups: u32,
+    pub resident_workgroups: u32,
+    pub tiles_per_wave: u32,
+    pub queue_class: u32,
+    pub classes_beside: u32,
+    pub reserved: u32,
+}
+
+#[repr(C)]
+#[derive(Clone, Copy, Debug, Default)]
+pub struct aic_residency_event {
+    pub kind: u32,
+    pub slot: u32,
+    pub running: u32,
+    pub reserved: u32,
+    pub start_ticks: u64,
+    pub end_ticks: u64,
 }
 
 #[repr(C)]
@@ -241,6 +265,8 @@
     pub fn aic_probe_expf(ctx: *mut aic_ctx, x: *const f32, n: u32, out: *mut f32) -> c_int;
     pub fn aic_probe_bloom(ctx: *mut aic_ctx, width: u32, height: u32, colorbuf: *const f32, exposure: f32, options: *const aic_options, out_rgba8: *mut u8, out_mip0: *mut u16, mip0_size: *mut u32) -> c_int;
     pub fn aic_probe_light_lut(ctx: *mut aic_ctx, out: *mut f32) -> c_int;
+    pub fn aic_probe_slot_residency(ctx: *mut aic_ctx, slot: u32, out: *mut aic_slot_residency) -> c_int;
+    pub fn aic_model_slot_residency(n_events: u32, events: *const aic_residency_event, out: *mut u32) -> c_int;
     pub fn aic_evaluate_light(ctx: *mut aic_ctx, layer: c_int, params: *const aic_light_params, info: *mut aic_light_info) -> c_int;
     pub fn aic_evaluate_light_submit(ctx: *mut aic_ctx, layer: c_int, params: *const aic_light_params) -> c_int;
     pub fn aic_evaluate_light_wait(ctx: *mut aic_ctx, layer: c_int, info: *mut aic_light_info) -> c_int;
```

Result: no change. 6272, median of 3 (+0.4%).
